# Alighieri1231/WaveformInversionUST

Hardware: NVIDIA B200
Metric: helmholtz_source_solves_per_sec (higher is better)
Workload: dtype c64

## Files before the change

waveforminversionust_b200/csrc/factor.cuh:

```cuda
#pragma once
#include "common.cuh"
#include "gemm_simt.cuh"
#include "gemm_tc2.cuh"
#include "gemm_tc2h.cuh"

namespace ust {

template <typename R>
struct FactorArgs {
    Geom g;
    int phase, step, nbatch;
    const cx<R>* planes;
    cx<R>* T;
    cx<R>* scratch;
    cx<R>* pbuf;
    int* status;
    uint16_t* Rp;
    uint16_t* Xp;
    uint16_t* Cp;
    uint16_t* Pp;
    uint16_t* Tp;
    size_t rp_stride;
    size_t rp2_stride;
    int kb;
// ... 628 lines not shown
    C* Pg = a.pbuf + (size_t)(a.zb0 + z) * GJ_NB * GJ_NB;
    for (int e = tid; e < GJ_NB * GJ_NB; e += 256) Pg[e] = A[(e & 63) * PV_LD + (e >> 6)];
}

template <typename R>
__global__ void __launch_bounds__(256, 1) gj_pivot_kernel(FactorArgs<R> a, int k, int form = 0) {
    extern __shared__ __align__(16) unsigned char smem_raw[];
    pdl_trigger();
    pdl_wait();
    if constexpr (sizeof(R) == 4) {
        if (a.Pp) { gj_pivot_blocked_global(a, k, blockIdx.z, smem_raw, threadIdx.x); return; }
        gj_pivot_body<R>(a, k, blockIdx.z, smem_raw, nullptr);
    } else {
        gj_pivot_blocked_f64(a, k, blockIdx.z, smem_raw, threadIdx.x, form);
    }
}

template <typename R>
constexpr size_t gj_rowpanel_smem() {
    return sizeof(R) == 8 ? 4 * sizeof(double) * GJ_NB * (GJ_NB + 8) : 2 * sizeof(cx<R>) * GJ_NB * GJ_NB;
}
template <typename R>
__global__ void __launch_bounds__(256) gj_rowpanel_kernel(FactorArgs<R> a, int k) {
    extern __shared__ __align__(16) unsigned char smem_raw[];
    const int z = blockIdx.z;
    const int row = chain_row(a.g, a.phase, z, a.step);
    if (row < 0) return;
    const int freq = (a.f0 + chain_freq(a.phase, z));
    const int nP = a.g.nP;
    const cx<R>* __restrict__ Xc = gj_buffer(a, z, freq, row, k);
    cx<R>* __restrict__ Xn = gj_buffer(a, z, freq, row, k + 1);
    const cx<R>* __restrict__ Pg = a.pbuf + (size_t)(a.zb0 + z) * GJ_NB * GJ_NB;
    const int k0 = k * GJ_NB, j0 = blockIdx.x * GJ_NB;
    const int tid = threadIdx.x;
    if constexpr (sizeof(R) == 8) {
        constexpr int LD = GJ_NB + 8;
        double(*Gr)[LD] = reinterpret_cast<double(*)[LD]>(smem_raw);
        double(*Gi)[LD] = Gr + GJ_NB;
        double(*Tr)[LD] = Gi + GJ_NB;
        double(*Ti)[LD] = Tr + GJ_NB;
        for (int e = tid; e < GJ_NB * GJ_NB; e += 256) {
            const int r = e / GJ_NB, c = e % GJ_NB;
            const cx<R> g = Pg[e];
            Gr[r][c] = g.re; Gi[r][c] = g.im;
            cx<R> tv;
            if (j0 == k0) tv = (r == c) ? cxone<R>() : cxzero<R>();
            else tv = Xc[(size_t)(k0 + r) * nP + j0 + c];
            Tr[r][c] = tv.re; Ti[r][c] = tv.im;
        }
        __syncthreads();
        const int lane = tid & 31, warp = tid >> 5;
        const int wm = (warp & 1) * 32, wn = (warp >> 1) * 16, fr = lane >> 2, fk = lane & 3;
        double cr[4][2][2], ci[4][2][2];
#pragma unroll
        for (int i = 0; i < 4; ++i)
#pragma unroll
            for (int j = 0; j < 2; ++j) { cr[i][j][0] = cr[i][j][1] = 0.0; ci[i][j][0] = ci[i][j][1] = 0.0; }
#pragma unroll 4
        for (int k4 = 0; k4 < GJ_NB; k4 += 4) {
            double ar[4], ai[4], br[2], bi[2], nbi[2];
#pragma unroll
            for (int i = 0; i < 4; ++i) { ar[i] = Gr[k4 + fk][wm + 8 * i + fr]; ai[i] = Gi[k4 + fk][wm + 8 * i + fr]; }
#pragma unroll
            for (int j = 0; j < 2; ++j) { br[j] = Tr[k4 + fk][wn + 8 * j + fr]; bi[j] = Ti[k4 + fk][wn + 8 * j + fr]; nbi[j] = -bi[j]; }
#pragma unroll
            for (int i = 0; i < 4; ++i)
#pragma unroll
                for (int j = 0; j < 2; ++j) {
                    dmma884(cr[i][j][0], cr[i][j][1], ar[i], br[j]);
                    dmma884(cr[i][j][0], cr[i][j][1], ai[i], nbi[j]);
                    dmma884(ci[i][j][0], ci[i][j][1], ar[i], bi[j]);
                    dmma884(ci[i][j][0], ci[i][j][1], ai[i], br[j]);
                }
        }
#pragma unroll
        for (int i = 0; i < 4; ++i)
#pragma unroll
            for (int j = 0; j < 2; ++j)
#pragma unroll
                for (int q = 0; q < 2; ++q)
                    Xn[(size_t)(k0 + wm + 8 * i + fr) * nP + j0 + wn + 8 * j + 2 * fk + q] = cx<R>(cr[i][j][q], ci[i][j][q]);
        return;
    } else {
    cx<R>(*G)[GJ_NB] = reinterpret_cast<cx<R>(*)[GJ_NB]>(smem_raw);
    cx<R>(*Tl)[GJ_NB] = reinterpret_cast<cx<R>(*)[GJ_NB]>(smem_raw + sizeof(cx<R>) * GJ_NB * GJ_NB);
    for (int e = tid; e < GJ_NB * GJ_NB; e += 256) {
        int r = e / GJ_NB, c = e % GJ_NB;
        G[r][c] = Pg[e];
        cx<R> tv;
        if (j0 == k0) tv = (r == c) ? cxone<R>() : cxzero<R>();
        else tv = Xc[(size_t)(k0 + r) * nP + j0 + c];
        Tl[r][c] = tv;
    }
    __syncthreads();
    const int tx = tid & 15, ty = tid >> 4;
    cx<R> acc[4][4];
#pragma unroll
    for (int i = 0; i < 4; ++i)
#pragma unroll
        for (int jj = 0; jj < 4; ++jj) acc[i][jj] = cxzero<R>();
#pragma unroll 8
    for (int kk = 0; kk < GJ_NB; ++kk) {
        cx<R> av[4], bv[4];
#pragma unroll
        for (int c = 0; c < 2; ++c) {
            av[2 * c] = G[kk][c * 32 + ty * 2];
            av[2 * c + 1] = G[kk][c * 32 + ty * 2 + 1];
            bv[2 * c] = Tl[kk][c * 32 + tx * 2];
            bv[2 * c + 1] = Tl[kk][c * 32 + tx * 2 + 1];
        }
#pragma unroll
        for (int i = 0; i < 4; ++i)
#pragma unroll
            for (int jj = 0; jj < 4; ++jj) cmac(acc[i][jj], av[i], bv[jj]);
    }
#pragma unroll
    for (int i = 0; i < 4; ++i) {
        int r = (i >> 1) * 32 + ty * 2 + (i & 1);
#pragma unroll
        for (int jj = 0; jj < 4; ++jj) {
            int c = (jj >> 1) * 32 + tx * 2 + (jj & 1);
            Xn[(size_t)(k0 + r) * nP + j0 + c] = acc[i][jj];
        }
    }
    }
}

template <typename R>
__global__ void __launch_bounds__(256) gj_update_kernel(FactorArgs<R> a, int k) {
    __shared__ GemmSmem<R, GJ_NB, GJ_NB> sm;
    const int z = blockIdx.z;
    const int row = chain_row(a.g, a.phase, z, a.step);
    if (row < 0) return;
    const int freq = (a.f0 + chain_freq(a.phase, z));
    const int nP = a.g.nP;
    const cx<R>* Xc = gj_buffer(a, z, freq, row, k);
    cx<R>* Xn = gj_buffer(a, z, freq, row, k + 1);
    const int ib = blockIdx.y + (blockIdx.y >= k ? 1 : 0);
    GemmTile<R> t;
    t.A = Xc + k * GJ_NB; t.lda = nP;
    t.B = Xn + (size_t)k * GJ_NB * nP; t.ldb = nP;
    t.Cin = Xc; t.ldcin = nP;
    t.Cout = Xn; t.ldc = nP;
    t.M = nP; t.N = nP; t.K = GJ_NB; t.Mstore = nP;
    t.m0 = ib * GJ_NB; t.n0 = blockIdx.x * GJ_NB;
    t.mask_lo = k * GJ_NB; t.mask_hi = (k + 1) * GJ_NB;
    t.sgn = R(-1);
    cgemm_tile<R, GJ_NB, GJ_NB, false>(t, sm);
}

__device__ __forceinline__ void gj_colsplit_body(const FactorArgs<float>& a, int k, int z, int bx, int tid) {
    const int row = chain_row(a.g, a.phase, z, a.step);
    if (row < 0) return;
    const int freq = (a.f0 + chain_freq(a.phase, z));
    const int nP = a.g.nP;
    const cx<float>* __restrict__ Xc = gj_buffer(a, z, freq, row, k);
    const int I = bx * 4 + (tid >> 6), J = (tid >> 3) & 7, r = tid & 7;
    const int rr = I * 8 + r;
    if (rr >= nP) return;
    const cx<float>* src = Xc + (size_t)rr * nP + k * GJ_NB + J * 8;
    float re[8], im[8];
#pragma unroll
    for (int c = 0; c < 8; ++c) { cx<float> v = src[c]; re[c] = v.re; im[c] = v.im; }
    uint32_t wr[3][4], wi[3][4];
#pragma unroll
    for (int qd = 0; qd < 4; ++qd) {
        tc::Split3 sr = tc::split2(re[2 * qd], re[2 * qd + 1]);
        tc::Split3 si = tc::split2(im[2 * qd], im[2 * qd + 1]);
#pragma unroll
        for (int sp = 0; sp < 3; ++sp) { wr[sp][qd] = sr.w[sp]; wi[sp][qd] = si.w[sp]; }
    }
    const size_t plane = (size_t)nP * GJ_NB;
    uint16_t* dst = a.Cp + ((size_t)(k & 1) * a.nbmax + a.zb0 + z) * tc2::NPL_A * plane + ((size_t)I * 8 + J) * 64 + r * 8;
#pragma unroll
    for (int sp = 0; sp < 3; ++sp) {
        *reinterpret_cast<uint4*>(dst + sp * plane) = make_uint4(wr[sp][0], wr[sp][1], wr[sp][2], wr[sp][3]);
        *reinterpret_cast<uint4*>(dst + (3 + sp) * plane) = make_uint4(wi[sp][0], wi[sp][1], wi[sp][2], wi[sp][3]);
    }
}

__device__ __forceinline__ void gj_rowsplit_body(const FactorArgs<float>& a, int k, int z, int tn, int r);
__device__ __forceinline__ void gj_colsplit_body(const FactorArgs<float>& a, int k, int z, int bx, int tid);
__global__ void __launch_bounds__(256) gj_k0_kernel(FactorArgs<float> a, int nrow, int ncol, int snap11) {
    extern __shared__ __align__(16) unsigned char smem_raw[];
    pdl_trigger();
    pdl_wait();
    const int z = blockIdx.z, bx = blockIdx.x;
    if (bx < nrow) {
        if (threadIdx.x < 128) gj_rowsplit_body(a, 0, z, bx, threadIdx.x);
    } else if (bx < nrow + ncol) {
        gj_colsplit_body(a, 0, z, bx - nrow, threadIdx.x);
    } else if (snap11 && bx == nrow + ncol) {
        const int row = chain_row(a.g, a.phase, z, a.step);
        if (row < 0) return;
        const int freq = a.f0 + chain_freq(a.phase, z), nP = a.g.nP;
        const cx<float>* __restrict__ Xc = gj_buffer(a, z, freq, row, 0);
        cx<float>* __restrict__ S = a.snap + ((size_t)a.nbmax + a.zb0 + z) * GJ_NB * GJ_NB;
        constexpr int PER = GJ_NB * GJ_NB / 2 / 256;
        float4 v[PER];
#pragma unroll
        for (int j = 0; j < PER; ++j) {
            const int w = threadIdx.x + 256 * j, r = w >> 5, c2 = w & 31;
            v[j] = *reinterpret_cast<const float4*>(Xc + (size_t)(GJ_NB + r) * nP + GJ_NB + 2 * c2);
        }
#pragma unroll
        for (int j = 0; j < PER; ++j) reinterpret_cast<float4*>(S)[threadIdx.x + 256 * j] = v[j];
    } else {
        gj_pivot_blocked_global(a, 0, z, smem_raw, threadIdx.x);
    }
}

__device__ __forceinline__ void gj_rowsplit_body(const FactorArgs<float>& a, int k, int z, int tn, int r) {
    const int row = chain_row(a.g, a.phase, z, a.step);
    if (row < 0) return;
    const int freq = (a.f0 + chain_freq(a.phase, z));
    const int nP = a.g.nP;
    const cx<float>* __restrict__ Xc = gj_buffer(a, z, freq, row, k);
    const int k0 = k * GJ_NB;
    const int n = tn * tc2::TN + r;
    uint16_t* base = a.Xp + ((size_t)(k & 1) * a.nbmax + a.zb0 + z) * a.rp_stride;
    for (int kg = 0; kg < 8; ++kg) {
        float re[8], im[8];
#pragma unroll
        for (int c = 0; c < 8; ++c) {
            cx<float> v = cxzero<float>();
            if (n < nP) {
                if (n >= k0 && n < k0 + GJ_NB) v = cx<float>((n - k0 == 8 * kg + c) ? 1.f : 0.f, 0.f);
                else v = Xc[(size_t)(k0 + 8 * kg + c) * nP + n];
            }
            re[c] = v.re; im[c] = v.im;
        }
        tc2::store_b8(base + ((size_t)tn * (GJ_NB / tc2::KC) + (kg >> 1)) * (tc2::B_STAGE / 2), r, kg & 1, re, im);
    }
}

__device__ __forceinline__ void gj_emit_a(const FactorArgs<float>& a, tc2::Tc2Tile& t, int z, int freq, int row, int k, int row_off) {
    const int nP = a.g.nP, nblk = nP / GJ_NB;
    t.ea_row_off = row_off;
    if (k + 1 < nblk) {
        const size_t plane = (size_t)nP * GJ_NB;
        t.ea_planes = a.Cp + ((size_t)((k + 1) & 1) * a.nbmax + a.zb0 + z) * tc2::NPL_A * plane;
        t.ea_plane_elems = (unsigned)plane; t.ea_nbc = GJ_NB / 8;
        t.ea_n_lo = (k + 1) * GJ_NB; t.ea_n_hi = (k + 2) * GJ_NB; t.ea_col_off = (k + 1) * GJ_NB;
        t.ea_zero_from = 0x7fffffff;
    } else {
        const size_t mat = (size_t)freq * a.g.M + row;
        t.ea_planes = a.Tp + mat * (size_t)tc2::NPL_A * nP * nP;
        t.ea_plane_elems = (unsigned)(nP * nP); t.ea_nbc = nP / 8;
        t.ea_n_lo = 0; t.ea_n_hi = nP; t.ea_col_off = 0;
        t.ea_zero_from = a.g.nI;
    }
}

__device__ __forceinline__ void gj_rowpanel_tile(const FactorArgs<float>& a, int k, int z, int row, int freq, int ntile, float bias_fix,
                                                 const CUtensorMap* pmap, unsigned char* tc2_smem, unsigned long long* trace = nullptr) {
    const int nP = a.g.nP;
    tc2::Tc2Tile t;
    tc2::tile_no_emit(t);
    t.bplanes = a.Xp + ((size_t)(k & 1) * a.nbmax + a.zb0 + z) * a.rp_stride;
    t.amat = (a.pp ? (k & 1) * a.nbmax : 0) + a.zb0 + z;
    t.Cin = nullptr; t.ldcin = nP;
    t.Cout = gj_buffer(a, z, freq, row, k + 1) + (size_t)k * GJ_NB * nP; t.ldc = nP;
    t.M = GJ_NB; t.N = nP; t.K = GJ_NB; t.Mstore = GJ_NB;
    t.m0 = 0; t.n0 = ntile * tc2::TNH;
    t.mask_lo = 0; t.mask_hi = 0; t.skip_lo = 0; t.skip_hi = 0;
    t.sgn = 1.f;
    t.bias_fix = bias_fix;
    t.drain_every = a.gj_drain;
    t.eb_planes = gj_rp(a, k, z); t.eb_m_lo = 0; t.eb_id_lo = 0; t.eb_id_hi = 0;
    gj_emit_a(a, t, z, freq, row, k, k * GJ_NB);
    t.trace = trace;
    tc2::cgemm_tile_h(t, pmap, tc2_smem);
}

__global__ void __launch_bounds__(tc2::NUM_THREADS_H, 2)
tc2_gj_rowpanel_kernel(FactorArgs<float> a, int k, float bias_fix, const __grid_constant__ CUtensorMap pmap) {
    extern __shared__ __align__(1024) unsigned char tc2_smem[];
    constexpr int TW = tc2::TNH;
    pdl_trigger();
    const int z = blockIdx.z;
    const int row = chain_row(a.g, a.phase, z, a.step);
    if (row < 0) { pdl_wait(); return; }
    const int freq = (a.f0 + chain_freq(a.phase, z));
    const int nP = a.g.nP;
    if (blockIdx.x * TW >= nP) {
        pdl_wait();
        const cx<float>* __restrict__ Xc = gj_buffer(a, z, freq, row, k);
        cx<float>* __restrict__ S = a.snap + (size_t)(a.zb0 + z) * GJ_NB * GJ_NB;
        const int k1 = (k + 1) * GJ_NB;
        constexpr int PER = GJ_NB * GJ_NB / 2 / 256;
        float4 v[PER];
#pragma unroll
        for (int j = 0; j < PER; ++j) {
            const int w = threadIdx.x + 256 * j, r = w >> 5, c2 = w & 31;
            v[j] = *reinterpret_cast<const float4*>(Xc + (size_t)(k1 + r) * nP + k1 + 2 * c2);
        }
#pragma unroll
        for (int j = 0; j < PER; ++j) reinterpret_cast<float4*>(S)[threadIdx.x + 256 * j] = v[j];
        return;
    }
    gj_rowpanel_tile(a, k, z, row, freq, blockIdx.x, bias_fix, &pmap, tc2_smem);
}

__global__ void __launch_bounds__(tc2::NUM_THREADS_H, 2)
tc2_gj_update_kernel(FactorArgs<float> a, int k, float bias_fix, int pivot_next, int rp_next, const __grid_constant__ CUtensorMap cmap,
                     const __grid_constant__ CUtensorMap pmap) {
    extern __shared__ __align__(1024) unsigned char tc2_smem[];
    constexpr int TW = tc2::TNH;
    pdl_trigger();
    int bid = blockIdx.x;
    if (pivot_next) {
        if (bid < a.nbatch) {
            {
                static_assert(tc2::CH_LD == GJ_NB + 1, "pivot body reads the staged tile with row stride GJ_NB + 1");
                const int z = bid, kb = k + 1, nP = a.g.nP;
                const int row = chain_row(a.g, a.phase, z, a.step);
                if (row < 0 || (a.exp & 2)) {
                    if (row >= 0 && rp_next && threadIdx.x == 0) atomicExch(gj_flag(a, 0, kb, z), 1);
                    pdl_wait();
                    return;
                }
                tc2::Tc2Tile t;
                tc2::tile_no_emit(t);
                t.bplanes = gj_rp(a, k, z);
                t.amat = (k & 1) * a.nbmax + a.zb0 + z;
                const cx<float>* S1 = a.snap + ((size_t)(a.pp ? (kb & 1) * a.nbmax : 0) + a.zb0 + z) * GJ_NB * GJ_NB;
                t.Cin = S1 - (size_t)(kb * GJ_NB) * GJ_NB - kb * GJ_NB; t.ldcin = GJ_NB;
                t.Cout = nullptr; t.ldc = nP; t.keep = 1;
                t.M = nP; t.N = nP; t.K = GJ_NB; t.Mstore = nP;
                t.m0 = (kb >> 1) * tc2::TM; t.n0 = kb * GJ_NB;
                t.mask_lo = 0; t.mask_hi = 0;
                t.skip_lo = (kb ^ 1) * GJ_NB; t.skip_hi = t.skip_lo + GJ_NB;
                t.sgn = -1.f; t.bias_fix = bias_fix; t.drain_every = a.gj_drain;
                const bool traced = a.trace && a.step == a.trace_step && k == a.trace_k && z < 24;
                if (traced) {
                    t.trace = a.trace + 16 * (1000 + z);
                    if (threadIdx.x == 0) { unsigned smid; asm volatile("mov.u32 %0, %%smid;" : "=r"(smid)); a.trace[16 * 1024 + 1000 + z] = smid; }
                }
                tc2::cgemm_tile_h(t, &cmap, tc2_smem);
                __syncthreads();
                if (a.exp & 1) {
                    if (rp_next && threadIdx.x == 0) atomicExch(gj_flag(a, 0, kb, z), 1);
                    return;
                }
                unsigned char* smem_al = tc2_smem + ((128u - (tc::smem_u32(tc2_smem) & 127u)) & 127u);
                cx<float>* blk = reinterpret_cast<cx<float>*>(smem_al) + (size_t)(kb & 1) * GJ_NB * tc2::CH_LD;
                cx<float>* scr = reinterpret_cast<cx<float>*>(smem_al) + (size_t)tc2::TM * tc2::CH_LD;
                static_assert((size_t)tc2::TM * tc2::CH_LD * sizeof(cx<float>) + gj_pivot2_scratch_bytes <= (size_t)tc2::STAGES_H * tc2::STAGE_H,
                              "pivot scratch must fit behind the staging tile inside the operand ring");
                FactorArgs<float> a2 = a;
                if (a.pp) a2.Pp = a.Pp + (size_t)(kb & 1) * a.nbmax * tc2::NPL_A * GJ_NB * GJ_NB;
                gj_pivot_blocked(a2, z, blk, scr, threadIdx.x, traced ? a.trace + 18 * 1024 + 16 * z : nullptr);
                if (traced && threadIdx.x == 0) a.trace[17 * 1024 + 1000 + z] = tc2::gtime();
                if (rp_next) {
                    __threadfence();
                    __syncthreads();
                    if (threadIdx.x == 0) atomicExch(gj_flag(a, 0, kb, z), 1);
                }
            }
            return;
        }
        bid -= a.nbatch;
    }
    const int nP = a.g.nP, nblk = nP / GJ_NB;
    const int tiles_m = (nP + tc2::TM - 1) / tc2::TM, tiles = (nP + TW - 1) / TW;
    const int ntile_ctas = a.nbatch * tiles_m * tiles;
    if (bid >= ntile_ctas) {
        const int idx = bid - ntile_ctas, z = idx / tiles, ntile = idx % tiles, kn = k + 1;
        const int row = chain_row(a.g, a.phase, z, a.step);
        if (row < 0) { pdl_wait(); return; }
        const int freq = a.f0 + chain_freq(a.phase, z);
        const bool traced = a.trace && a.step == a.trace_step && k == a.trace_k && idx < 96;
        if (traced && threadIdx.x == 0) {
            unsigned smid; asm volatile("mov.u32 %0, %%smid;" : "=r"(smid));
            a.trace[16 * 1024 + 900 + idx] = smid; a.trace[17 * 1024 + 900 + idx] = tc2::gtime();
        }
        pdl_wait();
        if (threadIdx.x == 0) {
            const int* fp = gj_flag(a, 0, kn, z);
            const int* fc = gj_flag(a, 1, kn, z);
            unsigned spins = 0;
            while (ld_acquire_gpu(fp) == 0 || ld_acquire_gpu(fc) < tiles) {
                __nanosleep(100);
                if (++spins > (1u << 22)) __trap();
            }
        }
        __syncthreads();
        asm volatile("fence.proxy.async;" ::: "memory");
        gj_rowpanel_tile(a, kn, z, row, freq, ntile, bias_fix, &pmap, tc2_smem, traced ? a.trace + 16 * (900 + idx) : nullptr);
        return;
    }
    int z, mt, nt;
    const int first = (k + 1) >> 1;
    if (rp_next) {
        const int mt_local = bid / (a.nbatch * tiles), rem = bid % (a.nbatch * tiles);
        z = rem / tiles; nt = rem % tiles;
        mt = mt_local == 0 ? first : (mt_local <= first ? mt_local - 1 : mt_local);
    } else {
        z = bid / (tiles_m * tiles);
        const int rem = bid % (tiles_m * tiles);
        mt = rem / tiles; nt = rem % tiles;
    }
    const int row = chain_row(a.g, a.phase, z, a.step);
    if (row < 0) { pdl_wait(); return; }
    const int freq = (a.f0 + chain_freq(a.phase, z));
    tc2::Tc2Tile t;
    tc2::tile_no_emit(t);
    t.bplanes = gj_rp(a, k, z);
    t.amat = (k & 1) * a.nbmax + a.zb0 + z;
    t.Cin = gj_buffer(a, z, freq, row, k); t.ldcin = nP;
    t.Cout = gj_buffer(a, z, freq, row, k + 1); t.ldc = nP;
    t.M = nP; t.N = nP; t.K = GJ_NB; t.Mstore = nP;
    t.m0 = mt * tc2::TM; t.n0 = nt * TW;
    t.mask_lo = k * GJ_NB; t.mask_hi = (k + 1) * GJ_NB;
    t.skip_lo = k * GJ_NB; t.skip_hi = (k + 1) * GJ_NB;
    t.sgn = -1.f;
    t.bias_fix = bias_fix;
    t.drain_every = a.gj_drain;
    gj_emit_a(a, t, z, freq, row, k, 0);
    if (k + 1 < nblk) {
        t.eb_planes = a.Xp + ((size_t)((k + 1) & 1) * a.nbmax + a.zb0 + z) * a.rp_stride;
        t.eb_m_lo = (k + 1) * GJ_NB; t.eb_id_lo = (k + 1) * GJ_NB; t.eb_id_hi = (k + 2) * GJ_NB;
    }
    if (a.trace && a.step == a.trace_step && k == a.trace_k && bid < 900) {
        t.trace = a.trace + 16 * bid;
        if (threadIdx.x == 0) { unsigned smid; asm volatile("mov.u32 %0, %%smid;" : "=r"(smid)); a.trace[16 * 1024 + bid] = smid; }
    }
    t.prefetch_cin = a.prefetch_cin;
    const int kk = k + 2;
    const bool snap_next = a.pp && kk < nblk && t.m0 == (kk >> 1) * tc2::TM && t.n0 == kk * GJ_NB;
    if (snap_next) t.keep = 1;
    tc2::cgemm_tile_h(t, &cmap, tc2_smem);
    if (snap_next) {
        __syncthreads();
        unsigned char* smem_al = tc2_smem + ((128u - (tc::smem_u32(tc2_smem) & 127u)) & 127u);
        const cx<float>* blk = reinterpret_cast<const cx<float>*>(smem_al) + (size_t)(kk & 1) * GJ_NB * tc2::CH_LD;
        cx<float>* __restrict__ S = a.snap + ((size_t)(kk & 1) * a.nbmax + a.zb0 + z) * GJ_NB * GJ_NB;
#pragma unroll
        for (int j = 0; j < GJ_NB * GJ_NB / tc2::NUM_THREADS_H; ++j) {
            const int e = threadIdx.x + tc2::NUM_THREADS_H * j;
            S[e] = blk[(e >> 6) * tc2::CH_LD + (e & 63)];
        }
    }
    if (rp_next && mt == first) {
        __threadfence();
        __syncthreads();
        if (threadIdx.x == 0) atomicAdd(gj_flag(a, 1, k + 1, z), 1);
    }
}

__global__ void __launch_bounds__(tc2::NUM_THREADS_H, 2)
tc2_gj_pivot_deep_kernel(FactorArgs<float> a, int j, float bias_fix, const __grid_constant__ CUtensorMap pmap, const __grid_constant__ CUtensorMap cmap) {
    extern __shared__ __align__(1024) unsigned char tc2_smem[];
    static_assert(tc2::CH_LD == GJ_NB + 1, "the pivot inversion reads the staged tile with row stride GJ_NB + 1");
    pdl_trigger();
    const int z = blockIdx.x, k = j - 1, nP = a.g.nP;
    const int row = chain_row(a.g, a.phase, z, a.step);
    if (row < 0) { pdl_wait(); return; }
    uint16_t* Rs = a.Rs + (size_t)(a.zb0 + z) * a.rp_stride;
    {
        tc2::Tc2Tile t;
        tc2::tile_no_emit(t);
        t.bplanes = a.Xp + ((size_t)(k & 1) * a.nbmax + a.zb0 + z) * a.rp_stride;
        t.amat = (k & 1) * a.nbmax + a.zb0 + z;
        t.Cin = nullptr; t.ldcin = nP;
        t.Cout = nullptr; t.ldc = nP;
        t.M = GJ_NB; t.N = nP; t.K = GJ_NB; t.Mstore = GJ_NB;
        t.m0 = 0; t.n0 = j * GJ_NB;
        t.mask_lo = 0; t.mask_hi = 0; t.skip_lo = 0; t.skip_hi = 0;
        t.sgn = 1.f; t.bias_fix = bias_fix; t.drain_every = a.gj_drain;
        t.eb_planes = Rs; t.eb_m_lo = 0; t.eb_id_lo = 0; t.eb_id_hi = 0;
        t.tmem_hold = 2;
        tc2::cgemm_tile_h(t, &pmap, tc2_smem);
    }
    __threadfence();
    asm volatile("fence.proxy.async;" ::: "memory");
    __syncthreads();
    tc2::engine_h_release(tc2_smem);
    {
        tc2::Tc2Tile t;
        tc2::tile_no_emit(t);
        t.bplanes = Rs;
        t.amat = (k & 1) * a.nbmax + a.zb0 + z;
        const cx<float>* S1 = a.snap + ((size_t)(j & 1) * a.nbmax + a.zb0 + z) * GJ_NB * GJ_NB;
        t.Cin = S1 - (size_t)(j * GJ_NB) * GJ_NB - j * GJ_NB; t.ldcin = GJ_NB;
        t.Cout = nullptr; t.ldc = nP; t.keep = 1;
        t.M = nP; t.N = nP; t.K = GJ_NB; t.Mstore = nP;
        t.m0 = (j >> 1) * tc2::TM; t.n0 = j * GJ_NB;
        t.mask_lo = 0; t.mask_hi = 0;
        t.skip_lo = (j ^ 1) * GJ_NB; t.skip_hi = t.skip_lo + GJ_NB;
        t.sgn = -1.f; t.bias_fix = bias_fix; t.drain_every = a.gj_drain;
        t.tmem_hold = 1;
        tc2::cgemm_tile_h(t, &cmap, tc2_smem);
    }
    __syncthreads();
    unsigned char* smem_al = tc2_smem + ((128u - (tc::smem_u32(tc2_smem) & 127u)) & 127u);
    cx<float>* blk = reinterpret_cast<cx<float>*>(smem_al) + (size_t)(j & 1) * GJ_NB * tc2::CH_LD;
    cx<float>* scr = reinterpret_cast<cx<float>*>(smem_al) + (size_t)tc2::TM * tc2::CH_LD;
    FactorArgs<float> a2 = a;
    a2.Pp = a.Pp + (size_t)(j & 1) * a.nbmax * tc2::NPL_A * GJ_NB * GJ_NB;
    gj_pivot_blocked(a2, z, blk, scr, threadIdx.x);
}

constexpr int GJ_KB = 128;
enum Gj2Mode { GJ2_MINI = 0, GJ2_FIXA = 1, GJ2_TRAIL = 2 };

__device__ __forceinline__ uint16_t* gj2_cp(const FactorArgs<float>& a, int K, int z) {
    return a.Cp + ((size_t)(K & 1) * a.nbmax + a.zb0 + z) * tc2::NPL_A * (size_t)a.g.nP * GJ_KB;
}
__device__ __forceinline__ void gj2_emit_next(const FactorArgs<float>& a, tc2::Tc2Tile& t, int z, int freq, int row, int K, int row_off) {
    const int nP = a.g.nP, nouter = nP / GJ_KB;
    t.ea_row_off = row_off;
    if (K + 1 < nouter) {
        t.ea_planes = gj2_cp(a, K + 1, z);
        t.ea_plane_elems = (unsigned)(nP * GJ_KB); t.ea_nbc = GJ_KB / 8;
        t.ea_n_lo = (K + 1) * GJ_KB; t.ea_n_hi = (K + 2) * GJ_KB; t.ea_col_off = (K + 1) * GJ_KB;
        t.ea_zero_from = 0x7fffffff;
    } else {
        const size_t mat = (size_t)freq * a.g.M + row;
        t.ea_planes = a.Tp + mat * (size_t)tc2::NPL_A * nP * nP;
        t.ea_plane_elems = (unsigned)(nP * nP); t.ea_nbc = nP / 8;
        t.ea_n_lo = 0; t.ea_n_hi = nP; t.ea_col_off = 0;
        t.ea_zero_from = a.g.nI;
    }
}

__device__ __forceinline__ void gj2_colsplit_body(const FactorArgs<float>& a, int z, int bx, int tid) {
    const int row = chain_row(a.g, a.phase, z, a.step);
    if (row < 0) return;
    const int freq = a.f0 + chain_freq(a.phase, z);
    const int nP = a.g.nP;
    const cx<float>* __restrict__ Xc = gj_buffer(a, z, freq, row, 0);
    const int I = bx * 2 + (tid >> 7), J = (tid >> 3) & 15, r = tid & 7;
    const int rr = I * 8 + r;
    if (rr >= nP) return;
    const cx<float>* src = Xc + (size_t)rr * nP + J * 8;
    float re[8], im[8];
#pragma unroll
    for (int c = 0; c < 8; ++c) { cx<float> v = src[c]; re[c] = v.re; im[c] = v.im; }
    const size_t plane = (size_t)nP * GJ_KB;
    tc2::store_a8(gj2_cp(a, 0, z) + ((size_t)I * (GJ_KB / 8) + J) * 64 + r * 8, plane, re, im);
}

__global__ void __launch_bounds__(256) gj2_k0_kernel(FactorArgs<float> a, int nrow, int ncol) {
    extern __shared__ __align__(16) unsigned char smem_raw[];
    pdl_trigger();
    pdl_wait();
    const int z = blockIdx.z, bx = blockIdx.x;
    if (bx < nrow) {
        if (threadIdx.x < 128) gj_rowsplit_body(a, 0, z, bx, threadIdx.x);
    } else if (bx < nrow + ncol) {
        gj2_colsplit_body(a, z, bx - nrow, threadIdx.x);
    } else {
        gj_pivot_blocked_global(a, 0, z, smem_raw, threadIdx.x);
    }
}

__global__ void __launch_bounds__(tc2::NUM_THREADS_H, 2)
tc2_gj2_rowpanel_kernel(FactorArgs<float> a, int k, float bias_fix, const __grid_constant__ CUtensorMap pmap) {
    extern __shared__ __align__(1024) unsigned char tc2_smem[];
    constexpr int TW = tc2::TNH;
    pdl_trigger();
    const int z = blockIdx.z;
    const int row = chain_row(a.g, a.phase, z, a.step);
    if (row < 0) { pdl_wait(); return; }
    const int freq = a.f0 + chain_freq(a.phase, z);
    const int nP = a.g.nP, K = k >> 1;
    if (blockIdx.x * TW >= nP) {
        pdl_wait();
        const cx<float>* __restrict__ Xc = gj_buffer(a, z, freq, row, k);
        cx<float>* __restrict__ S = a.snap + (size_t)(a.zb0 + z) * GJ_NB * GJ_NB;
        const int k1 = (k + 1) * GJ_NB;
        constexpr int PER = GJ_NB * GJ_NB / 2 / 256;
        float4 v[PER];
#pragma unroll
        for (int j = 0; j < PER; ++j) {
            const int w = threadIdx.x + 256 * j, r = w >> 5, c2 = w & 31;
            v[j] = *reinterpret_cast<const float4*>(Xc + (size_t)(k1 + r) * nP + k1 + 2 * c2);
        }
#pragma unroll
        for (int j = 0; j < PER; ++j) reinterpret_cast<float4*>(S)[threadIdx.x + 256 * j] = v[j];
        return;
    }
    tc2::Tc2Tile t;
    tc2::tile_no_emit(t);
    t.bplanes = a.Xp + ((size_t)(k & 1) * a.nbmax + a.zb0 + z) * a.rp_stride;
    t.amat = a.zb0 + z;
    t.Cin = nullptr; t.ldcin = nP;
    t.Cout = gj_buffer(a, z, freq, row, k) + (size_t)k * GJ_NB * nP; t.ldc = nP;
    t.M = GJ_NB; t.N = nP; t.K = GJ_NB; t.Mstore = GJ_NB;
    t.m0 = 0; t.n0 = blockIdx.x * TW;
    t.mask_lo = 0; t.mask_hi = 0; t.skip_lo = 0; t.skip_hi = 0;
    t.sgn = 1.f;
    t.bias_fix = bias_fix;
    t.drain_every = a.gj_drain;
    t.eb_planes = a.Rp + (size_t)(a.zb0 + z) * a.rp2_stride; t.eb_m_lo = 0; t.eb_id_lo = 0; t.eb_id_hi = 0;
    t.eb_chunks = GJ_KB / tc2::KC; t.eb_chunk0 = (k & 1) * (GJ_NB / tc2::KC);
    if ((k & 1) == 0) {
        t.ea_row_off = k * GJ_NB;
        t.ea_planes = gj2_cp(a, K, z);
        t.ea_plane_elems = (unsigned)(nP * GJ_KB); t.ea_nbc = GJ_KB / 8;
        t.ea_n_lo = (k + 1) * GJ_NB; t.ea_n_hi = (k + 2) * GJ_NB; t.ea_col_off = k * GJ_NB;
        t.ea_zero_from = 0x7fffffff;
    } else {
        gj2_emit_next(a, t, z, freq, row, K, k * GJ_NB);
    }
    tc2::cgemm_tile_h(t, &pmap, tc2_smem);
}

__global__ void __launch_bounds__(tc2::NUM_THREADS_H, 2)
tc2_gj2_update_kernel(FactorArgs<float> a, int k, int mode, float bias_fix, int pivot_next, const __grid_constant__ CUtensorMap cmap) {
    extern __shared__ __align__(1024) unsigned char tc2_smem[];
    constexpr int TW = tc2::TNH;
    pdl_trigger();
    const int nP = a.g.nP, nblk = nP / GJ_NB, K = k >> 1;
    const int ka = 2 * K, kbk = 2 * K + 1;
    int bid = blockIdx.x;
    if (pivot_next) {
        if (bid < a.nbatch) {
            static_assert(tc2::CH_LD == GJ_NB + 1, "the pivot inversion reads the staged tile with row stride GJ_NB + 1");
            const int z = bid, kn = mode == GJ2_MINI ? k + 1 : ka + 2;
            const int row = chain_row(a.g, a.phase, z, a.step);
            if (row < 0 || (a.exp & 2)) { pdl_wait(); return; }
            tc2::Tc2Tile t;
            tc2::tile_no_emit(t);
            t.bplanes = a.Rp + (size_t)(a.zb0 + z) * a.rp2_stride;
            t.b_chunks = GJ_KB / tc2::KC; t.b_chunk0 = 0;
            t.amat = (K & 1) * a.nbmax + a.zb0 + z; t.a_k0 = 0;
            const cx<float>* S1 = a.snap + (size_t)(a.zb0 + z) * GJ_NB * GJ_NB;
            t.Cin = S1 - (size_t)(kn * GJ_NB) * GJ_NB - kn * GJ_NB; t.ldcin = GJ_NB;
            t.Cout = nullptr; t.ldc = nP; t.keep = 1;
            t.M = nP; t.N = nP; t.K = mode == GJ2_MINI ? GJ_NB : GJ_KB; t.Mstore = nP;
            t.m0 = (kn >> 1) * tc2::TM; t.n0 = kn * GJ_NB;
            t.mask_lo = 0; t.mask_hi = 0;
            t.skip_lo = (kn ^ 1) * GJ_NB; t.skip_hi = t.skip_lo + GJ_NB;
            t.sgn = -1.f; t.bias_fix = bias_fix; t.drain_every = a.gj_drain;
            tc2::cgemm_tile_h(t, &cmap, tc2_smem);
            __syncthreads();
            if (a.exp & 1) return;
            unsigned char* smem_al = tc2_smem + ((128u - (tc::smem_u32(tc2_smem) & 127u)) & 127u);
            cx<float>* blk = reinterpret_cast<cx<float>*>(smem_al) + (size_t)(kn & 1) * GJ_NB * tc2::CH_LD;
            cx<float>* scr = reinterpret_cast<cx<float>*>(smem_al) + (size_t)tc2::TM * tc2::CH_LD;
            gj_pivot_blocked(a, z, blk, scr, threadIdx.x);
            return;
        }
        bid -= a.nbatch;
    }
    const int tiles = nP / TW, tiles_m = nP / tc2::TM;
    const int mt_count = mode == GJ2_TRAIL ? tiles_m - 1 : 1;
    const int z = bid / (mt_count * tiles), rem = bid % (mt_count * tiles);
    const int row = chain_row(a.g, a.phase, z, a.step);
    if (row < 0) { pdl_wait(); return; }
    const int freq = a.f0 + chain_freq(a.phase, z);
    int mt = rem / tiles;
    if (mode == GJ2_TRAIL) mt += (mt >= K) ? 1 : 0;
    else mt = K;
    tc2::Tc2Tile t;
    tc2::tile_no_emit(t);
    t.bplanes = a.Rp + (size_t)(a.zb0 + z) * a.rp2_stride;
    t.b_chunks = GJ_KB / tc2::KC;
    t.amat = (K & 1) * a.nbmax + a.zb0 + z;
    t.Cin = gj_buffer(a, z, freq, row, k); t.ldcin = nP;
    t.Cout = gj_buffer(a, z, freq, row, k + 1); t.ldc = nP;
    t.M = nP; t.N = nP; t.Mstore = nP;
    t.m0 = mt * tc2::TM; t.n0 = (rem % tiles) * TW;
    t.sgn = -1.f;
    t.bias_fix = bias_fix;
    t.drain_every = a.gj_drain;
    t.prefetch_cin = a.prefetch_cin;
    if (mode == GJ2_MINI) {
        t.K = GJ_NB; t.a_k0 = 0; t.b_chunk0 = 0;
        t.mask_lo = ka * GJ_NB; t.mask_hi = (ka + 1) * GJ_NB;
        t.skip_lo = ka * GJ_NB; t.skip_hi = (ka + 1) * GJ_NB;
        t.eb_planes = a.Xp + ((size_t)(kbk & 1) * a.nbmax + a.zb0 + z) * a.rp_stride;
        t.eb_m_lo = kbk * GJ_NB; t.eb_id_lo = kbk * GJ_NB; t.eb_id_hi = (kbk + 1) * GJ_NB;
    } else if (mode == GJ2_FIXA) {
        t.K = GJ_NB; t.a_k0 = GJ_NB; t.b_chunk0 = GJ_NB / tc2::KC;
        t.mask_lo = kbk * GJ_NB; t.mask_hi = (kbk + 1) * GJ_NB;
        t.skip_lo = kbk * GJ_NB; t.skip_hi = (kbk + 1) * GJ_NB;
        t.eb_planes = a.Rp + (size_t)(a.zb0 + z) * a.rp2_stride;
        t.eb_chunks = GJ_KB / tc2::KC; t.eb_chunk0 = 0;
        t.eb_m_lo = ka * GJ_NB; t.eb_id_lo = 0; t.eb_id_hi = 0;
        gj2_emit_next(a, t, z, freq, row, K, 0);
    } else {
        t.K = GJ_KB; t.a_k0 = 0; t.b_chunk0 = 0;
        t.mask_lo = ka * GJ_NB; t.mask_hi = (ka + 2) * GJ_NB;
        t.skip_lo = 0; t.skip_hi = 0;
        if (ka + 2 < nblk) {
            t.eb_planes = a.Xp + ((size_t)((ka + 2) & 1) * a.nbmax + a.zb0 + z) * a.rp_stride;
            t.eb_m_lo = (ka + 2) * GJ_NB; t.eb_id_lo = (ka + 2) * GJ_NB; t.eb_id_hi = (ka + 3) * GJ_NB;
        }
        gj2_emit_next(a, t, z, freq, row, K, 0);
    }
    tc2::cgemm_tile_h(t, &cmap, tc2_smem);
}

}
```

waveforminversionust_b200/csrc/gemm_tc2h.cuh:

```cuda
#pragma once
#include "gemm_tc2.cuh"

namespace ust {
namespace tc2 {

constexpr int TNH = 64;
constexpr int BH_PLANE = 2 * TNH * KC * 2;
constexpr int BH_STAGE = NPL_B * BH_PLANE;
constexpr int STAGE_H = A_STAGE + BH_STAGE;
constexpr int STAGES_H = 3;
constexpr int NUM_THREADS_H = 256;
constexpr int NUM_WARPS_H = 8;
constexpr int CH_LD = TNH + 1;
constexpr int SMEM_BYTES_H = STAGES_H * STAGE_H + 128 + 128 + 384;
static_assert(TM * CH_LD * 8 <= STAGES_H * STAGE_H, "epilogue staging tile must fit in the operand ring");
static_assert(2 * (SMEM_BYTES_H + 1024) <= 227 * 1024, "two CTAs per SM");
constexpr uint32_t TMEM_COLS_H = 256;
constexpr uint32_t IDESC_N64 = IDESC_BASE | ((64u >> 3) << 17);

__device__ __forceinline__ void engine_h_release(unsigned char* smem_raw) {
    __syncthreads();
    if (threadIdx.x == 0) {
        const uint32_t smem_base = (smem_u32(smem_raw) + 127u) & ~127u;
        const uint32_t bar_base = smem_base + STAGES_H * STAGE_H;
        for (int i = 0; i < 2 * STAGES_H + 3; ++i) asm volatile("mbarrier.inval.shared::cta.b64 [%0];" ::"r"(bar_base + 8u * i) : "memory");
    }
    __syncthreads();
}

__device__ __forceinline__ void cgemm_tile_h(const Tc2Tile& t_in, const CUtensorMap* amap, unsigned char* smem_raw) {
    typedef cx<float> C;
    const int tid = threadIdx.x, warp = tid >> 5, lane = tid & 31;
    if (warp == 0) TC2_TRACE(0);
    if (tid == 0) asm volatile("prefetch.tensormap [%0];" ::"l"((uint64_t)amap) : "memory");
    const uint32_t smem_base = (smem_u32(smem_raw) + 127u) & ~127u;
    unsigned char* smem_al = smem_raw + (smem_base - smem_u32(smem_raw));
    const uint32_t bar_base = smem_base + STAGES_H * STAGE_H;
    auto full_bar = [&](int s) { return bar_base + 8u * s; };
    auto empty_bar = [&](int s) { return bar_base + 8u * (STAGES_H + s); };
    const uint32_t d1_full = bar_base + 8u * (2 * STAGES_H);
    const uint32_t d1_empty = bar_base + 8u * (2 * STAGES_H + 1);
    const uint32_t d2_full = bar_base + 8u * (2 * STAGES_H + 2);
    const uint32_t tmem_slot = bar_base + 8u * (2 * STAGES_H + 3);
    volatile uint32_t* tmem_slot_ptr = reinterpret_cast<volatile uint32_t*>(smem_al + (tmem_slot - smem_base));
    Tc2Tile* t_sh = reinterpret_cast<Tc2Tile*>(smem_al + STAGES_H * STAGE_H + 128);
    if (tid == 0) *t_sh = t_in;
    const Tc2Tile& t = *t_sh;

    if (warp == 2) {
        if (lane == 0) {
            for (int s = 0; s < STAGES_H; ++s) { mbar_init(full_bar(s), 1); mbar_init(empty_bar(s), 2); }
            mbar_init(d1_full, 1);
            mbar_init(d1_empty, NUM_WARPS_H);
            mbar_init(d2_full, 1);
            asm volatile("fence.mbarrier_init.release.cluster;" ::: "memory");
        }
        __syncwarp();
        if (!(t_in.tmem_hold & 1)) {
            asm volatile("tcgen05.alloc.cta_group::1.sync.aligned.shared::cta.b32 [%0], %1;" ::"r"(tmem_slot), "r"(TMEM_COLS_H) : "memory");
            asm volatile("tcgen05.relinquish_alloc_permit.cta_group::1.sync.aligned;" ::: "memory");
        }
    }
    asm volatile("tcgen05.fence::before_thread_sync;" ::: "memory");
    __syncthreads();
    asm volatile("tcgen05.fence::after_thread_sync;" ::: "memory");
    const uint32_t tmem_acc = *tmem_slot_ptr;
    pdl_wait();
    if (warp == 0) TC2_TRACE(1);
    const uint32_t D1 = tmem_acc, D2 = tmem_acc + 2 * TNH;
    const int nk = (t.K + KC - 1) / KC;
    const int D = t.drain_every < 1 ? 1 : (t.drain_every > nk ? nk : t.drain_every);

    const int bch = t.b_chunks > 0 ? t.b_chunks : nk;
    const unsigned char* bsrc = reinterpret_cast<const unsigned char*>(t.bplanes) + ((size_t)(t.n0 / TN) * bch + t.b_chunk0) * B_STAGE + ((t.n0 % TN) / TNH) * 2048;
    const int am0 = t.m0, amat = t.amat, ak0 = t.a_k0;
    auto load_chunk = [&](int c) {
        const int s = c % STAGES_H;
        const uint32_t sa = smem_base + s * STAGE_H, sb = sa + A_STAGE;
        mbar_expect_tx_e(full_bar(s), STAGE_H);
        tma_load_5d_e(sa, amap, full_bar(s), 0, (ak0 + c * KC) >> 3, am0 >> 3, 0, amat);
        const unsigned char* bc = bsrc + (size_t)c * B_STAGE;
#pragma unroll
        for (int p = 0; p < NPL_B; ++p) {
            bulk_load_e(sb + p * BH_PLANE, bc + p * B_PLANE, 2048, full_bar(s));
            bulk_load_e(sb + p * BH_PLANE + 2048, bc + p * B_PLANE + 4096, 2048, full_bar(s));
        }
    };
    if (warp == 0) {
        load_chunk(0);
        TC2_TRACE(2);
    } else if (warp == 2) {
        for (int c = 1; c < nk && c < STAGES_H; ++c) load_chunk(c);
    }
    if (t.Cin && tid >= 128 && t.prefetch_cin) {
        const int rr = tid - 128, m = t.m0 + rr;
        const int ncols = t.N - t.n0 < TNH ? t.N - t.n0 : TNH;
        if (m < t.Mstore && !(m >= t.skip_lo && m < t.skip_hi) && ncols > 0 && ((ncols * 8) & 15) == 0 && ((t.ldcin & 1) == 0) && ((t.n0 & 1) == 0))
            asm volatile("cp.async.bulk.prefetch.L2.global [%0], %1;" ::"l"((uint64_t)(t.Cin + (size_t)m * t.ldcin + t.n0)), "r"((uint32_t)(ncols * 8)) : "memory");
    }

    const uint32_t id1 = IDESC_N128, id2 = IDESC_N64 | IDESC_ANEG, id3 = IDESC_N64;
    uint64_t dAr[3], dAi[3], dB[3], dBi[3];
#pragma unroll
    for (int i = 0; i < 3; ++i) {
        dAr[i] = make_desc(smem_base + i * A_PLANE, 128u, 256u);
        dAi[i] = make_desc(smem_base + (3 + i) * A_PLANE, 128u, 256u);
        dB[i] = make_desc(smem_base + A_STAGE + i * BH_PLANE, 128u, 256u);
        dBi[i] = make_desc(smem_base + A_STAGE + i * BH_PLANE + (TNH / 8) * 256, 128u, 256u);
    }
    auto issue = [&](uint32_t d, uint64_t so, int i, int j, uint32_t acc_first) {
        umma_e(d, dAr[i] + so, dB[j] + so, id1, acc_first);
        umma_e(d, dAi[i] + so, dBi[j] + so, id2, 1u);
        umma_e(d + TNH, dAi[i] + so, dB[j] + so, id3, 1u);
    };

    const int q = warp & 3, cg = warp >> 2;
    const uint32_t lane_addr = ((uint32_t)(q * 32)) << 16;
    float acc_re[32], acc_im[32];
#pragma unroll
    for (int j = 0; j < 32; ++j) { acc_re[j] = 0.f; acc_im[j] = 0.f; }

    for (int c = 0; c < nk; ++c) {
        const int s = c % STAGES_H;
        const uint32_t use = (uint32_t)(c / STAGES_H);
        if (warp < 2) {
            const uint64_t so = (uint64_t)((uint32_t)(s * STAGE_H) >> 4);
            mbar_wait(full_bar(s), use & 1u);
            if (warp == 0) {
                if (c == 0) TC2_TRACE(3);
                if (c > 0 && c % D == 0) mbar_wait(d1_empty, (uint32_t)(c / D - 1) & 1u);
                if (c == nk - 1) TC2_TRACE(8);
                asm volatile("tcgen05.fence::after_thread_sync;" ::: "memory");
                issue(D1, so, 0, 0, c % D == 0 ? 0u : 1u);
                if ((c + 1) % D == 0 || c == nk - 1) umma_commit_e(d1_full);
                umma_commit_e(empty_bar(s));
                if (c == 0) TC2_TRACE(4);
            } else {
                asm volatile("tcgen05.fence::after_thread_sync;" ::: "memory");
                issue(D2, so, 0, 1, c > 0 ? 1u : 0u);
                issue(D2, so, 1, 0, 1u);
                issue(D2, so, 0, 2, 1u);
                issue(D2, so, 2, 0, 1u);
                issue(D2, so, 1, 1, 1u);
                umma_commit_e(empty_bar(s));
                if (c == nk - 1) { TC2_TRACE(9); umma_commit_e(d2_full); }
            }
            __syncwarp();
        }
        if ((c + 1) % D == 0 || c == nk - 1) {
        mbar_wait(d1_full, (uint32_t)(c / D) & 1u);
        if (warp == 3 && c == 0) TC2_TRACE(5);
        asm volatile("tcgen05.fence::after_thread_sync;" ::: "memory");
#pragma unroll
        for (int h = 0; h < 4; ++h) {
            uint32_t vr[8], vi[8];
            tmem_ld8(D1 + lane_addr + (uint32_t)(32 * cg + 8 * h), vr);
            tmem_ld8(D1 + lane_addr + (uint32_t)(TNH + 32 * cg + 8 * h), vi);
            asm volatile("tcgen05.wait::ld.sync.aligned;" ::: "memory");
            if (h == 3) {
                asm volatile("tcgen05.fence::before_thread_sync;" ::: "memory");
                __syncwarp();
                if (lane == 0) mbar_arrive(d1_empty);
                if (warp == 3 && c == 0) TC2_TRACE(6);
            }
#pragma unroll
            for (int j = 0; j < 8; ++j) {
                acc_re[8 * h + j] += __uint_as_float(vr[j]);
                acc_im[8 * h + j] += __uint_as_float(vi[j]);
            }
        }
        }
        if (warp == 0 && c + STAGES_H < nk) {
            mbar_wait(empty_bar(s), use & 1u);
            load_chunk(c + STAGES_H);
        }
    }
    mbar_wait(d2_full, 0);
    if (warp == 3) TC2_TRACE(10);
    asm volatile("tcgen05.fence::after_thread_sync;" ::: "memory");
    C* stage = reinterpret_cast<C*>(smem_al);
    {
        const int r = q * 32 + lane;
        const float bias = t.bias_fix * (float)D;
#pragma unroll
        for (int h = 0; h < 4; ++h) {
            uint32_t vr[8], vi[8];
            tmem_ld8(D2 + lane_addr + (uint32_t)(32 * cg + 8 * h), vr);
            tmem_ld8(D2 + lane_addr + (uint32_t)(TNH + 32 * cg + 8 * h), vi);
            asm volatile("tcgen05.wait::ld.sync.aligned;" ::: "memory");
#pragma unroll
            for (int j = 0; j < 8; ++j) {
                const float ar = acc_re[8 * h + j], ai = acc_im[8 * h + j];
                const float cr = fmaf(ar, bias, __uint_as_float(vr[j]));
                const float ci = fmaf(ai, bias, __uint_as_float(vi[j]));
                stage[(size_t)r * CH_LD + 32 * cg + 8 * h + j] = C(ar + cr, ai + ci);
            }
        }
    }
    if (warp == 3) TC2_TRACE(11);
    asm volatile("tcgen05.fence::before_thread_sync;" ::: "memory");
    __syncthreads();
    if (warp == 2 && !(t_in.tmem_hold & 2)) {
        asm volatile("tcgen05.fence::after_thread_sync;" ::: "memory");
        asm volatile("tcgen05.dealloc.cta_group::1.sync.aligned.b32 %0, %1;" ::"r"(tmem_acc), "r"(TMEM_COLS_H) : "memory");
    }
    if (warp == 3) TC2_TRACE(15);
    const Tc2Tile tl = *t_sh;
    const bool emit = tl.ea_planes != nullptr || tl.eb_planes != nullptr || tl.keep;
    const bool vec_ok = ((tl.ldc & 1) == 0) && ((((uintptr_t)tl.Cout) & 15) == 0) && (tl.n0 % 2 == 0) &&
                        (!tl.Cin || (((tl.ldcin & 1) == 0) && ((((uintptr_t)tl.Cin) & 15) == 0)));
    if (vec_ok && tl.n0 + TNH <= tl.N) {
        constexpr int RPW = TM / NUM_WARPS_H;
        float4 cin[RPW];
        unsigned live = 0;
        const int nloc = lane * 2, n = tl.n0 + nloc;
#pragma unroll
        for (int j = 0; j < RPW; ++j) {
            const int m = tl.m0 + warp + NUM_WARPS_H * j;
            const bool lv = m < tl.Mstore && !(m >= tl.skip_lo && m < tl.skip_hi);
            live |= (lv ? 1u : 0u) << j;
            cin[j] = make_float4(0.f, 0.f, 0.f, 0.f);
            if (lv && tl.Cin) cin[j] = *reinterpret_cast<const float4*>(tl.Cin + (size_t)m * tl.ldcin + n);
        }
        const bool z0 = n >= tl.mask_lo && n < tl.mask_hi, z1 = n + 1 >= tl.mask_lo && n + 1 < tl.mask_hi;
#pragma unroll
        for (int j = 0; j < RPW; ++j) {
            const int rr = warp + NUM_WARPS_H * j;
            const int m = tl.m0 + rr;
            if (!((live >> j) & 1u)) continue;
            const C a0 = stage[(size_t)rr * CH_LD + nloc], a1 = stage[(size_t)rr * CH_LD + nloc + 1];
            float4 c = cin[j];
            if (z0) { c.x = 0.f; c.y = 0.f; }
            if (z1) { c.z = 0.f; c.w = 0.f; }
            c.x += tl.sgn * a0.re; c.y += tl.sgn * a0.im; c.z += tl.sgn * a1.re; c.w += tl.sgn * a1.im;
            if (tl.Cout) *reinterpret_cast<float4*>(tl.Cout + (size_t)m * tl.ldc + n) = c;
            if (emit) { stage[(size_t)rr * CH_LD + nloc] = C(c.x, c.y); stage[(size_t)rr * CH_LD + nloc + 1] = C(c.z, c.w); }
        }
    } else {
        for (int rr = warp; rr < TM; rr += NUM_WARPS_H) {
            const int m = tl.m0 + rr;
            if (m >= tl.Mstore || (m >= tl.skip_lo && m < tl.skip_hi)) continue;
            const int nloc = lane * 2, n = tl.n0 + nloc;
            if (n >= tl.N) continue;
            const C a0 = stage[(size_t)rr * CH_LD + nloc], a1 = stage[(size_t)rr * CH_LD + nloc + 1];
            C c0 = cxzero<float>(), c1 = cxzero<float>();
            if (tl.Cin) {
                const C* ci = tl.Cin + (size_t)m * tl.ldcin + n;
                c0 = ci[0];
                if (n + 1 < tl.N) c1 = ci[1];
                if (n >= tl.mask_lo && n < tl.mask_hi) c0 = cxzero<float>();
                if (n + 1 >= tl.mask_lo && n + 1 < tl.mask_hi) c1 = cxzero<float>();
            }
            c0.re += tl.sgn * a0.re; c0.im += tl.sgn * a0.im;
            c1.re += tl.sgn * a1.re; c1.im += tl.sgn * a1.im;
            if (tl.Cout) {
                C* co = tl.Cout + (size_t)m * tl.ldc + n;
                co[0] = c0;
                if (n + 1 < tl.N) co[1] = c1;
            }
            if (emit) { stage[(size_t)rr * CH_LD + nloc] = c0; stage[(size_t)rr * CH_LD + nloc + 1] = c1; }
        }
    }
    if (warp == 3) TC2_TRACE(12);
    if (emit) {
        __syncthreads();
        if (tl.eb_planes && tl.eb_m_lo >= tl.m0 && tl.eb_m_lo < tl.m0 + TM) {
            const int r0 = tl.eb_m_lo - tl.m0;
#pragma unroll
            for (int h = 0; h < 2; ++h) {
                const int e = tid + NUM_THREADS_H * h;
                const int nloc = e & (TNH - 1), kg = e >> 6;
                const int n = tl.n0 + nloc;
                float re[8], im[8];
#pragma unroll
                for (int c = 0; c < 8; ++c) {
                    C v = stage[(size_t)(r0 + 8 * kg + c) * CH_LD + nloc];
                    if (n >= tl.eb_id_lo && n < tl.eb_id_hi) v = C((n - tl.eb_id_lo == 8 * kg + c) ? 1.f : 0.f, 0.f);
                    if (n >= tl.N) v = cxzero<float>();
                    re[c] = v.re; im[c] = v.im;
                }
                const int ech = tl.eb_chunks > 0 ? tl.eb_chunks : 64 / KC;
                uint16_t* chunk = tl.eb_planes + ((size_t)(n / TN) * ech + tl.eb_chunk0 + (kg >> 1)) * (B_STAGE / 2);
                store_b8(chunk, n % TN, kg & 1, re, im);
            }
        }
        if (tl.ea_planes) {
            const int lo = tl.ea_n_lo > tl.n0 ? tl.ea_n_lo : tl.n0;
            const int hi = tl.ea_n_hi < tl.n0 + TNH ? tl.ea_n_hi : tl.n0 + TNH;
            const int nJ = hi > lo ? (hi - lo) >> 3 : 0;
            for (int e = tid; e < nJ * TM; e += NUM_THREADS_H) {
                const int rr = e & (TM - 1), jj = e >> 7;
                const int m = tl.m0 + rr;
                if (m >= tl.Mstore || (m >= tl.skip_lo && m < tl.skip_hi)) continue;
                const int n8 = lo + 8 * jj;
                const int tr = m + tl.ea_row_off, tcol = n8 - tl.ea_col_off;
                float re[8], im[8];
#pragma unroll
                for (int c = 0; c < 8; ++c) {
                    C v = stage[(size_t)rr * CH_LD + (n8 - tl.n0) + c];
                    if (tr >= tl.ea_zero_from || tcol + c >= tl.ea_zero_from || n8 + c >= tl.N) v = cxzero<float>();
                    re[c] = v.re; im[c] = v.im;
                }
                uint16_t* dst = tl.ea_planes + ((size_t)(tr >> 3) * tl.ea_nbc + (tcol >> 3)) * 64 + (tr & 7) * 8;
                store_a8(dst, tl.ea_plane_elems, re, im);
            }
        }
    }
    if (warp == 3) TC2_TRACE(13);
    if (warp == 2) TC2_TRACE(14);
}

}
}
```

waveforminversionust_b200/csrc/ustfwi.cu:

```cuda
#include "../../include/ustfwi.h"

#include <math.h>
#include <stdlib.h>
#include <string.h>

#include <algorithm>
#include <map>
#include <mutex>
#include <vector>

#include "assemble.cuh"
#include "common.cuh"
#include "factor.cuh"
#include "fwi.cuh"
#include "sweep.cuh"

namespace ust {
static thread_local std::string g_err;
thread_local long long g_launches = 0;
bool g_use_pdl = true;
thread_local bool g_pdl_batch_ok = true;
void set_error(const std::string& s) { g_err = s; }
}

using namespace ust;

struct ust_plan {
    ust_plan_desc d;
    Geom g;
    size_t rsz, csz;
    double h = 0, gr = 1, a0 = 0, Lpml = 0;
    bool grid_set = false, acq_set = false, factored = false;
    bool use_tc2 = false;
    bool t_ring = false;
    int prefetch_cin = 1;
    static constexpr int MAX_GROUPS = 8;
    int ngroups = 2;
    cudaStream_t side[MAX_GROUPS] = {};
    cudaEvent_t ev_fork = nullptr, ev_join[MAX_GROUPS] = {};
    bool deep = false;
    cudaStream_t pivst[MAX_GROUPS] = {};
    cudaEvent_t ev_upd[MAX_GROUPS] = {}, ev_piv[MAX_GROUPS][2] = {};
    uint16_t* Rs = nullptr;
    bool fuse = false;
    int* gj_flags = nullptr;
    uint16_t *Tp = nullptr, *Wp = nullptr;
    void* snap = nullptr;
    uint16_t *Rp = nullptr, *Cp = nullptr, *Xp = nullptr, *Pp = nullptr;
    size_t rp_stride = 0, rp2_stride = 0;
    bool gj2 = false;
    CUtensorMap cmaps[2], cmaps2[2], pmaps[2];
    size_t wp_stride = 0;
    int kpad = 0;
    int gj_drain = 1, sweep_drain = 1;
    float bias_fix = 2.5e-8f;
    CUtensorMap amaps[2];
    int nfreq_cur = 0;
    std::vector<double> freqs_cur;
    size_t bytes = 0;
    int num_sms = 148;
    void *exn = nullptr, *rexh = nullptr, *eyn = nullptr, *reyh = nullptr;
    double *d_vminmax = nullptr, *d_freqs = nullptr, *d_bde = nullptr, *d_scal = nullptr, *d_invv2 = nullptr;
    double* d_sig2 = nullptr;
    int* d_status = nullptr;
    void *planes = nullptr, *T = nullptr, *scratch = nullptr, *W = nullptr, *pbuf = nullptr;
    void *vel = nullptr, *U = nullptr, *Lam = nullptr, *src_est = nullptr, *Xh = nullptr;
    void *slow_h2d = nullptr, *rec_h2d = nullptr, *grad_d2h = nullptr;
    int *src_lin = nullptr, *rx_lin = nullptr, *mask = nullptr;
    int nt = 0, nelem = 0, nm = 0;
    bool onehot_ok = false;
    short first_row[8], last_row[8];
    void *slow_in = nullptr, *rec_in = nullptr, *grad_out = nullptr, *sd_in = nullptr;
    void *v_in = nullptr, *hv_out = nullptr, *drec = nullptr;
    void *kappa_in = nullptr, *grad_kappa_out = nullptr;
    void *kappa_h2d = nullptr, *grad_kappa_d2h = nullptr;
    bool fwi_done = false;
    bool lossy = false;
    bool gn_ok = false;
    bool use_graphs = true;
    struct GraphEntry { cudaGraphExec_t exec = nullptr; long long launches = 0; };
    std::map<long long, GraphEntry> graphs;
    cudaEvent_t ev_in = nullptr, ev_out = nullptr;
    double* h_stage = nullptr;
    cudaStream_t own_stream = nullptr;
    unsigned long long* trace = nullptr;
    int trace_step = -1, trace_k = -1;
    bool schur_pivot0 = true;
    int pdl_min_batch = 8;
    int active_groups = 1;
    int eval_nfreq = 1;
    int ksplit_ok = 2;
    int exp = 0;
    bool lookahead = true;
    bool prof = false;
    std::vector<cudaEvent_t> ev;
    std::vector<int> ev_cls;
    size_t ev_used = 0;
};

struct ProfScope {
    ust_plan* p; long idx; cudaStream_t st;
    ProfScope(ust_plan* p_, int cls, cudaStream_t st_) : p(p_), idx(-1), st(st_) {
        if (p->prof && p->ev_used + 2 <= p->ev.size()) {
            idx = (long)p->ev_used; p->ev_used += 2; p->ev_cls[idx / 2] = cls;
            cudaEventRecord(p->ev[idx], st);
        }
    }
    ~ProfScope() { if (idx >= 0) cudaEventRecord(p->ev[idx + 1], st); }
};
enum ProfClass { PC_ASSEMBLE = 0, PC_SCHUR, PC_GJ_PANEL, PC_GJ_UPDATE, PC_TRI_APPLY, PC_SWEEP_GEMM, PC_RECEIVER, PC_GRADIENT, PC_T_SPLIT, PC_GJ_PIVOT, PC_GJ_ROWPANEL, PC_GJ_K0, PC_COUNT };

static int dev_alloc(ust_plan* p, void** ptr, size_t bytes) {
    UST_CUDA(cudaMalloc(ptr, bytes));
    p->bytes += bytes;
    return 0;
}

static int check_plan(const ust_plan* p) {
    if (!p) { set_error("null plan"); return 1; }
    return 0;
}

static int dump_update_trace(ust_plan* p, cudaStream_t st) {
    std::vector<unsigned long long> h(19 * 1024);
    UST_CUDA(cudaStreamSynchronize(st));
    UST_CUDA(cudaMemcpy(h.data(), p->trace, h.size() * sizeof(unsigned long long), cudaMemcpyDeviceToHost));
    unsigned long long t0 = ~0ull;
    for (int b = 0; b < 1024; ++b) if (h[16 * b] && h[16 * b] < t0) t0 = h[16 * b];
    for (int b = 0; b < 1024; ++b) {
        if (!h[16 * b]) continue;
        fprintf(stderr, "upd cta %4d sm %3d:", b, (int)h[16 * 1024 + b]);
        for (int i = 0; i < 16; ++i) fprintf(stderr, " %lld", h[16 * b + i] ? (long long)(h[16 * b + i] - t0) : -1LL);
        fprintf(stderr, " %lld", h[17 * 1024 + b] ? (long long)(h[17 * 1024 + b] - t0) : -1LL);
        if (b >= 1000 && b < 1024)
            for (int i = 0; i < 13; ++i) fprintf(stderr, " %lld", h[18 * 1024 + 16 * (b - 1000) + i] ? (long long)(h[18 * 1024 + 16 * (b - 1000) + i] - t0) : -1LL);
        fprintf(stderr, "\n");
    }
    UST_CUDA(cudaMemset(p->trace, 0, h.size() * sizeof(unsigned long long)));
    return 0;
}

static void drop_graphs(ust_plan* p) {
    for (auto& kv : p->graphs)
        if (kv.second.exec) cudaGraphExecDestroy(kv.second.exec);
    p->graphs.clear();
}

template <typename R>
static int set_grid_impl(ust_plan* p, const double* x, const double* y, double a0, double L) {
    const int Nx = p->g.Nx, Ny = p->g.Ny;
    double h = (x[Nx - 1] - x[0]) / (Nx - 1), gh = (y[Ny - 1] - y[0]) / (Ny - 1);
    p->h = h; p->gr = gh / h; p->a0 = a0; p->Lpml = L;
    auto prof = [&](const double* c, int n, std::vector<cx<R>>& node, std::vector<cx<R>>& rhalf) {
        double cmin = c[0], cmax = c[n - 1];
        double ctr = 0.5 * (cmin + cmax), span = 0.5 * (cmax - cmin);
        node.resize(n); rhalf.resize(n);
        for (int i = 0; i < 2 * n - 1; ++i) {
            double xe = cmin + (cmax - cmin) * (double)i / (double)(2 * (n - 1));
            double s = fmax(fabs(xe - ctr) - span + L, 0.0) / L;
            double im = -a0 * s * s;
            if ((i & 1) == 0) node[i / 2] = cx<R>((R)1.0, (R)im);
            else {
                double d = 1.0 + im * im;
                rhalf[i / 2] = cx<R>((R)(1.0 / d), (R)(-im / d));
            }
        }
        rhalf[n - 1] = cx<R>((R)0, (R)0);
    };
    std::vector<cx<R>> exn, rexh, eyn, reyh;
    prof(x, Nx, exn, rexh);
    prof(y, Ny, eyn, reyh);
    UST_CUDA(cudaMemcpy(p->exn, exn.data(), Nx * sizeof(cx<R>), cudaMemcpyHostToDevice));
    UST_CUDA(cudaMemcpy(p->rexh, rexh.data(), Nx * sizeof(cx<R>), cudaMemcpyHostToDevice));
    UST_CUDA(cudaMemcpy(p->eyn, eyn.data(), Ny * sizeof(cx<R>), cudaMemcpyHostToDevice));
    UST_CUDA(cudaMemcpy(p->reyh, reyh.data(), Ny * sizeof(cx<R>), cudaMemcpyHostToDevice));
    p->grid_set = true;
    p->factored = false;
    return 0;
}

template <typename R>
static int gj_invert_batch(ust_plan* p, int phase, int step, int f0, int nf, cudaStream_t st, int gidx) {
    const Geom& g = p->g;
    const int nbatch = phase == PH_CHAIN ? 2 * nf : nf;
    FactorArgs<R> a;
    a.g = g; a.phase = phase; a.step = step; a.nbatch = nbatch;
    a.f0 = f0; a.zb0 = 2 * f0; a.t_ring = p->t_ring ? 1 : 0;
    ust::g_pdl_batch_ok = nbatch * p->active_groups > p->pdl_min_batch ||
                          (long long)nbatch * p->active_groups * cdiv_i(g.nP, tc2::TM) * (g.nP / tc2::TNH) > 2LL * p->num_sms;
    a.planes = (const cx<R>*)p->planes; a.T = (cx<R>*)p->T; a.scratch = (cx<R>*)p->scratch; a.pbuf = (cx<R>*)p->pbuf; a.status = p->d_status;
    a.Rp = p->Rp; a.Cp = p->Cp; a.Xp = p->Xp; a.Pp = p->Pp; a.Tp = p->Tp; a.rp_stride = p->rp_stride; a.nbmax = 2 * p->d.max_freq;
    a.rp2_stride = p->rp2_stride; a.kb = p->gj2 ? GJ_KB : GJ_NB;
    a.inplace = p->use_tc2 ? 1 : 0; a.gj_drain = p->gj_drain; a.snap = (cx<R>*)p->snap;
    a.trace = p->trace; a.trace_step = p->trace_step; a.trace_k = p->trace_k;
    a.prefetch_cin = p->prefetch_cin; a.exp = p->exp;
    a.deep = (p->deep && g.nP / GJ_NB > 1) ? 1 : 0; a.Rs = p->Rs;
    a.fuse = (p->fuse && !p->deep && p->lookahead && g.nP / GJ_NB > 1 && g.nP / GJ_NB <= GJ_MAXBLK) ? 1 : 0;
    a.pp = (a.deep || a.fuse) ? 1 : 0; a.flags = p->gj_flags;
    const int nblk = g.nP / GJ_NB;
    {
        dim3 grid(cdiv_i(g.nP, SchurTile<R>::TS), cdiv_i(g.nP, SchurTile<R>::TS), nbatch), block(16, 16);
        const int pivot0 = (sizeof(R) == 4 && p->use_tc2 && p->schur_pivot0) ? 1 : 0;
        ProfScope ps(p, PC_SCHUR, st);
        UST_CUDA(launch_pdl(schur_kernel<R>, grid, block, pivot0 ? gj_pivot2_scratch_bytes : 0, st, a, pivot0));
        UST_LAUNCH_CHECK();
    }
    const size_t smem = gj_rowpanel_smem<R>();
    if constexpr (sizeof(R) == 4) {
        if (p->use_tc2 && p->gj2) {
            {
                ProfScope ps(p, PC_GJ_K0, st);
                const int nrow = cdiv_i(g.nP, tc2::TN), ncol = g.nP / 16;
                UST_CUDA(launch_pdl(gj2_k0_kernel, dim3(nrow + ncol + (p->schur_pivot0 ? 0 : 1), 1, nbatch), dim3(256), gj_pivot2_smem_bytes, st, a, nrow, ncol));
            }
            UST_LAUNCH_CHECK();
            const int tiles_h = g.nP / tc2::TNH, tiles_m = g.nP / tc2::TM;
            auto rowpanel = [&](int k) -> int {
                if (p->exp & 4) return 0;
                ProfScope ps(p, PC_GJ_ROWPANEL, st);
                const int snap_cta = (k + 1 < nblk) ? 1 : 0;
                UST_CUDA(launch_pdl(tc2_gj2_rowpanel_kernel, dim3(tiles_h + snap_cta, 1, nbatch), dim3(tc2::NUM_THREADS_H), tc2::SMEM_BYTES_H, st, a, k, p->bias_fix, p->pmaps[0]));
                UST_LAUNCH_CHECK();
                return 0;
            };
            auto update = [&](int k, int mode, int mt_count, int pivot_next) -> int {
                ProfScope ps(p, mode == GJ2_TRAIL ? PC_GJ_UPDATE : (mode == GJ2_MINI ? PC_GJ_PANEL : PC_GJ_PIVOT), st);
                UST_CUDA(launch_pdl(tc2_gj2_update_kernel, dim3(nbatch * mt_count * tiles_h + (pivot_next ? nbatch : 0)), dim3(tc2::NUM_THREADS_H),
                                    tc2::SMEM_BYTES_H, st, a, k, mode, p->bias_fix, pivot_next, p->cmaps2[0]));
                UST_LAUNCH_CHECK();
                return 0;
            };
            for (int K = 0; K < nblk / 2; ++K) {
                const int ka = 2 * K, kbk = ka + 1;
                UST_TRY(rowpanel(ka));
                UST_TRY(update(ka, GJ2_MINI, 1, 1));
                UST_TRY(rowpanel(kbk));
                UST_TRY(update(kbk, GJ2_FIXA, 1, 0));
                if (tiles_m > 1) UST_TRY(update(ka, GJ2_TRAIL, tiles_m - 1, ka + 2 < nblk ? 1 : 0));
            }
            return 0;
        }
        if (p->use_tc2) {
            const bool deep = a.deep != 0;
            {
                ProfScope ps(p, PC_GJ_K0, st);
                const int nrow = cdiv_i(g.nP, tc2::TN), ncol = nblk > 1 ? cdiv_i(g.nP, 32) : 0;
                UST_CUDA(launch_pdl(gj_k0_kernel, dim3(nrow + ncol + (a.pp ? 1 : 0) + (p->schur_pivot0 ? 0 : 1), 1, nbatch), dim3(256), gj_pivot2_smem_bytes, st, a, nrow, ncol, a.pp));
            }
            UST_LAUNCH_CHECK();
            const bool la = p->lookahead && nblk > 1 && !deep;
            const int tiles = cdiv_i(g.nP, tc2::TN), tiles_h = cdiv_i(g.nP, tc2::TNH);
            cudaStream_t ps_st = p->pivst[gidx];
            auto pivot_deep = [&](int j) -> int {
                UST_CUDA(cudaEventRecord(p->ev_upd[gidx], st));
                UST_CUDA(cudaStreamWaitEvent(ps_st, p->ev_upd[gidx], 0));
                {
                    ProfScope p1(p, PC_GJ_PIVOT, ps_st);
                    UST_CUDA(launch_pdl(tc2_gj_pivot_deep_kernel, dim3(nbatch), dim3(tc2::NUM_THREADS_H), tc2::SMEM_BYTES_H, ps_st, a, j, p->bias_fix, p->pmaps[0], p->cmaps[0]));
                }
                UST_LAUNCH_CHECK();
                UST_CUDA(cudaEventRecord(p->ev_piv[gidx][j & 1], ps_st));
                return 0;
            };
            if (deep) UST_TRY(pivot_deep(1));
            for (int k = 0; k < nblk; ++k) {
                {
                    ProfScope ps(p, PC_GJ_PANEL, st);
                    if (k > 0 && !la && !deep) {
                        ProfScope p1(p, PC_GJ_PIVOT, st);
                        UST_CUDA(launch_pdl(gj_pivot_kernel<R>, dim3(1, 1, nbatch), dim3(256), gj_pivot2_smem_bytes, st, a, k, 0));
                        UST_LAUNCH_CHECK();
                    }
                    if (k > 0 && deep) UST_CUDA(cudaStreamWaitEvent(st, p->ev_piv[gidx][k & 1], 0));
                    if (!(p->exp & 4) && (!a.fuse || k == 0)) {
                        ProfScope p2(p, PC_GJ_ROWPANEL, st);
                        const int snap_cta = (la && !a.pp && k + 1 < nblk) ? 1 : 0;
                        UST_CUDA(launch_pdl(tc2_gj_rowpanel_kernel, dim3(tiles_h + snap_cta, 1, nbatch), dim3(tc2::NUM_THREADS_H), tc2::SMEM_BYTES_H, st, a, k, p->bias_fix, p->pmaps[0]));
                    }
                    UST_LAUNCH_CHECK();
                }
                if (nblk > 1) {
                    const int pivot_next = (la && k + 1 < nblk) ? 1 : 0;
                    const int rp_next = (a.fuse && k + 1 < nblk && !(p->exp & 4)) ? 1 : 0;
                    ProfScope ps(p, PC_GJ_UPDATE, st);
                    UST_CUDA(launch_pdl(tc2_gj_update_kernel, dim3(nbatch * tiles * tiles_h + (pivot_next ? nbatch : 0) + (rp_next ? nbatch * tiles_h : 0)), dim3(tc2::NUM_THREADS_H),
                                        tc2::SMEM_BYTES_H, st, a, k, p->bias_fix, pivot_next, rp_next, p->cmaps[0], p->pmaps[0]));
                    UST_LAUNCH_CHECK();
                }
                if (deep && k + 2 < nblk) UST_TRY(pivot_deep(k + 2));
            }
            return 0;
        }
    }
    const bool la64 = sizeof(R) == 8 && p->lookahead && nblk > 1 && p->pivst[gidx] != nullptr;
    const size_t piv_smem = sizeof(R) == 8 ? gj_pivot_f64_smem_bytes : gj_pivot_smem<R>();
    for (int k = 0; k < nblk; ++k) {
        {
            ProfScope ps(p, PC_GJ_PANEL, st);
            if (k == 0 || !la64) {
                ProfScope p1(p, PC_GJ_PIVOT, st);
                gj_pivot_kernel<R><<<dim3(1, 1, nbatch), 256, piv_smem, st>>>(a, k, 0);
            } else {
                UST_CUDA(cudaStreamWaitEvent(st, p->ev_piv[gidx][k & 1], 0));
            }
            UST_LAUNCH_CHECK();
            {
                ProfScope p2(p, PC_GJ_ROWPANEL, st);
                gj_rowpanel_kernel<R><<<dim3(nblk, 1, nbatch), 256, smem, st>>>(a, k);
            }
            UST_LAUNCH_CHECK();
        }
        if (la64 && k + 1 < nblk) {
            cudaStream_t ps_st = p->pivst[gidx];
            UST_CUDA(cudaEventRecord(p->ev_upd[gidx], st));
            UST_CUDA(cudaStreamWaitEvent(ps_st, p->ev_upd[gidx], 0));
            {
                ProfScope p1(p, PC_GJ_PIVOT, ps_st);
                gj_pivot_kernel<R><<<dim3(1, 1, nbatch), 256, piv_smem, ps_st>>>(a, k + 1, 1);
            }
            UST_LAUNCH_CHECK();
            UST_CUDA(cudaEventRecord(p->ev_piv[gidx][(k + 1) & 1], ps_st));
        }
        if (nblk > 1) {
            {
                ProfScope ps(p, PC_GJ_UPDATE, st);
                gj_update_kernel<R><<<dim3(nblk, nblk - 1, nbatch), 256, 0, st>>>(a, k);
            }
            UST_LAUNCH_CHECK();
        }
    }
    return 0;
}

static int upload_params(ust_plan* p, int nfreq, const double* freqs, const double* bde, cudaStream_t st) {
    if (!p->grid_set) { set_error("ust_factor: ust_plan_set_grid has not been called"); return 1; }
    if (nfreq < 1 || nfreq > p->d.max_freq) { set_error("ust_factor: nfreq out of range"); return 1; }
    UST_CUDA(cudaMemcpyAsync(p->d_freqs, freqs, nfreq * sizeof(double), cudaMemcpyHostToDevice, st));
    if (bde) UST_CUDA(cudaMemcpyAsync(p->d_bde, bde, 3 * nfreq * sizeof(double), cudaMemcpyHostToDevice, st));
    p->freqs_cur.assign(freqs, freqs + nfreq);
    return 0;
}

struct Group { int f0, nf; cudaStream_t st; int idx; };

static std::vector<Group> make_groups(ust_plan* p, int f_begin, int nfreq, cudaStream_t main_st, bool allow_split = true) {
    int G = std::min(std::min(p->ngroups, nfreq / 4), (int)ust_plan::MAX_GROUPS);
    if (p->prof || !allow_split || G < 1) G = 1;
    p->active_groups = G;
    p->eval_nfreq = nfreq;
    std::vector<Group> gs;
    for (int i = 0; i < G; ++i) {
        const int lo = (int)((long long)nfreq * i / G), hi = (int)((long long)nfreq * (i + 1) / G);
        gs.push_back({f_begin + lo, hi - lo, i == 0 ? main_st : p->side[i], i});
    }
    return gs;
}
static int fork_groups(ust_plan* p, const std::vector<Group>& gs) {
    if (gs.size() < 2) return 0;
    UST_CUDA(cudaEventRecord(p->ev_fork, gs[0].st));
    for (size_t i = 1; i < gs.size(); ++i) UST_CUDA(cudaStreamWaitEvent(gs[i].st, p->ev_fork, 0));
    return 0;
}
static int join_groups(ust_plan* p, const std::vector<Group>& gs) {
    for (size_t i = 1; i < gs.size(); ++i) {
        UST_CUDA(cudaEventRecord(p->ev_join[i], gs[i].st));
        UST_CUDA(cudaStreamWaitEvent(gs[0].st, p->ev_join[i], 0));
    }
    return 0;
}

template <typename R>
static int factor_prologue(ust_plan* p, const void* vel_dev, int nfreq, bool has_bde, cudaStream_t st, const void* kappa_dev = nullptr) {
    const Geom& g = p->g;
    if (!has_bde) {
        minmax_kernel<R><<<1, 1024, 0, st>>>((const R*)vel_dev, g.N, p->d_vminmax);
        UST_LAUNCH_CHECK();
        stencil_params_kernel<<<nfreq, 1024, 0, st>>>(p->d_vminmax, p->d_freqs, p->h, p->gr, p->d_bde);
        UST_LAUNCH_CHECK();
    }
    UST_CUDA(cudaMemsetAsync(p->d_status, 0, sizeof(int), st));
    if (kappa_dev) sig2_kernel<R><<<(unsigned)((g.N + 255) / 256), 256, 0, st>>>((const R*)vel_dev, (const R*)kappa_dev, (double2*)p->d_sig2, g.N);
    else inv_v2_kernel<R><<<(unsigned)((g.N + 255) / 256), 256, 0, st>>>((const R*)vel_dev, p->d_invv2, g.N);
    UST_LAUNCH_CHECK();
    return 0;
}

template <typename R>
static int factor_groups(ust_plan* p, const void* vel_dev, const std::vector<Group>& gs, bool lossy = false) {
    const Geom& g = p->g;
    AsmArgs aa;
    aa.g = g; aa.h = p->h; aa.gr = p->gr; aa.stencil = p->d.stencil; aa.exp = (p->exp & 8) ? 1 : 0;
    for (const Group& q : gs)
        for (int c0 = 0; c0 < q.nf; c0 += ASM_MAXF) {
            const int f0 = q.f0 + c0;
            aa.nfreq = std::min(q.nf - c0, (int)ASM_MAXF);
            ProfScope ps(p, PC_ASSEMBLE, q.st);
            const dim3 grid(cdiv_i(g.Nx, 256), g.Ny);
            if (lossy)
                assemble_kernel<R, true><<<grid, 256, 0, q.st>>>(
                    aa, p->d_sig2, (const cx<R>*)p->exn, (const cx<R>*)p->rexh, (const cx<R>*)p->eyn, (const cx<R>*)p->reyh,
                    p->d_freqs + f0, p->d_bde + 3 * f0, (cx<R>*)p->planes + (size_t)f0 * 9 * g.N);
            else
                assemble_kernel<R, false><<<grid, 256, 0, q.st>>>(
                    aa, p->d_invv2, (const cx<R>*)p->exn, (const cx<R>*)p->rexh, (const cx<R>*)p->eyn, (const cx<R>*)p->reyh,
                    p->d_freqs + f0, p->d_bde + 3 * f0, (cx<R>*)p->planes + (size_t)f0 * 9 * g.N);
            UST_LAUNCH_CHECK();
        }
    const int len = std::max(g.mid, g.M - 1 - g.mid);
    for (int s = 0; s < len; ++s)
        for (const Group& q : gs) UST_TRY(gj_invert_batch<R>(p, PH_CHAIN, s, q.f0, q.nf, q.st, q.idx));
    for (const Group& q : gs) UST_TRY(gj_invert_batch<R>(p, PH_MID, 0, q.f0, q.nf, q.st, q.idx));
    return 0;
}

template <typename R>
static int factor_enqueue(ust_plan* p, const void* vel_dev, int nfreq, bool has_bde, cudaStream_t st, const void* kappa_dev) {
    UST_TRY(factor_prologue<R>(p, vel_dev, nfreq, has_bde, st, kappa_dev));
    const std::vector<Group> gs = make_groups(p, 0, nfreq, st);
    UST_TRY(fork_groups(p, gs));
    UST_TRY(factor_groups<R>(p, vel_dev, gs, kappa_dev != nullptr));
    UST_TRY(join_groups(p, gs));
    p->nfreq_cur = nfreq;
    p->factored = true;
    return 0;
}

template <typename R>
static int factor_impl(ust_plan* p, const void* vel_dev, int nfreq, const double* freqs, const double* bde, cudaStream_t st,
                       const void* kappa_dev = nullptr) {
    p->gn_ok = false;
    UST_TRY(upload_params(p, nfreq, freqs, bde, st));
    if (kappa_dev) p->lossy = true;
    return factor_enqueue<R>(p, vel_dev, nfreq, bde != nullptr, st, kappa_dev);
}

template <typename R, int BM, int BN>
static int launch_sweep_gemm(ust_plan* p, const SweepArgs<R>& s, dim3 grid, cudaStream_t st) {
    {
        ProfScope ps(p, PC_SWEEP_GEMM, st);
        if (s.adjoint) sweep_gemm_kernel<R, BM, BN, true><<<grid, 256, 0, st>>>(s);
        else sweep_gemm_kernel<R, BM, BN, false><<<grid, 256, 0, st>>>(s);
    }
    UST_LAUNCH_CHECK();
    return 0;
}

template <typename R>
static int sweep_step(ust_plan* p, SweepArgs<R>& s, cudaStream_t st) {
    const Geom& g = p->g;
    const long long elems = (long long)g.nI * s.nrhs;
    ust::g_pdl_batch_ok = s.nbatch * p->active_groups > p->pdl_min_batch;
    if constexpr (sizeof(R) == 4) {
        if (p->use_tc2) {
            Tc2SweepExtra x;
            x.Wp = p->Wp + (size_t)2 * s.f0 * p->wp_stride;
            x.wp_stride = p->wp_stride; x.kpad = p->kpad; x.bias_fix = p->bias_fix; x.drain_every = p->sweep_drain;
            x.prefetch_cin = p->prefetch_cin; x.ksplit = 1;
            {
                ProfScope ps(p, PC_TRI_APPLY, st);
                UST_CUDA(launch_pdl(tri_apply2_kernel, dim3(p->kpad / 8, cdiv_i(s.nrhs, tc2::TN), s.nbatch), dim3(128), 0, st, s, x));
            }
            UST_LAUNCH_CHECK();
            dim3 grid(cdiv_i(s.nrhs, tc2::TN), cdiv_i(g.nI, tc2::TM), s.nbatch);
            const long long all_tiles = 2LL * p->eval_nfreq * grid.x * grid.y;
            const int nchunks = p->kpad / tc2::KC;
            x.ksplit = 1;
            if (p->ksplit_ok >= 2 && 2 * all_tiles <= p->num_sms && nchunks >= 8) x.ksplit = 2;
            if (p->ksplit_ok >= 4 && 4 * all_tiles <= p->num_sms && nchunks >= 16) x.ksplit = 4;
            {
                ProfScope ps(p, PC_SWEEP_GEMM, st);
                if (x.ksplit > 1) {
                    grid.x *= x.ksplit;
                    if (s.adjoint) UST_CUDA(launch_pdl_cluster(tc2_sweep_gemm_kernel<true>, grid, dim3(tc2::NUM_THREADS), tc2::SMEM_BYTES, st, (unsigned)x.ksplit, s, x, p->amaps[1]));
                    else UST_CUDA(launch_pdl_cluster(tc2_sweep_gemm_kernel<false>, grid, dim3(tc2::NUM_THREADS), tc2::SMEM_BYTES, st, (unsigned)x.ksplit, s, x, p->amaps[0]));
                } else if (s.adjoint) UST_CUDA(launch_pdl(tc2_sweep_gemm_kernel<true>, grid, dim3(tc2::NUM_THREADS), tc2::SMEM_BYTES, st, s, x, p->amaps[1]));
                else UST_CUDA(launch_pdl(tc2_sweep_gemm_kernel<false>, grid, dim3(tc2::NUM_THREADS), tc2::SMEM_BYTES, st, s, x, p->amaps[0]));
            }
            UST_LAUNCH_CHECK();
            return 0;
        }
    }
    {
        ProfScope ps(p, PC_TRI_APPLY, st);
        tri_apply_kernel<R><<<dim3((unsigned)((elems + 255) / 256), 1, s.nbatch), 256, 0, st>>>(s);
    }
    UST_LAUNCH_CHECK();
    const int bn = s.nrhs > 32 ? 64 : 32;
    int bm = 64;
    if ((long long)cdiv_i(g.nI, 64) * cdiv_i(s.nrhs, bn) * s.nbatch < p->num_sms) bm = 32;
    dim3 grid(cdiv_i(s.nrhs, bn), cdiv_i(g.nI, bm), s.nbatch);
    if (bm == 64 && bn == 64) return launch_sweep_gemm<R, 64, 64>(p, s, grid, st);
    if (bm == 32 && bn == 64) return launch_sweep_gemm<R, 32, 64>(p, s, grid, st);
    if (bm == 64 && bn == 32) return launch_sweep_gemm<R, 64, 32>(p, s, grid, st);
    return launch_sweep_gemm<R, 32, 32>(p, s, grid, st);
}

template <typename R>
static int sweeps_groups(ust_plan* p, const std::vector<Group>& gs, cx<R>* X, size_t x_stride, int nrhs, int adjoint, bool onehot = false) {
    const Geom& g = p->g;
    std::vector<SweepArgs<R>> sv(gs.size());
    for (size_t i = 0; i < gs.size(); ++i) {
        SweepArgs<R>& s = sv[i];
        const int f0 = gs[i].f0;
        s.g = g; s.adjoint = adjoint; s.nrhs = nrhs;
        s.onehot = (onehot && p->onehot_ok) ? 1 : 0;
        for (int j = 0; j < 8; ++j) { s.first_row[j] = p->first_row[j]; s.last_row[j] = p->last_row[j]; }
        s.planes = (const cx<R>*)p->planes + (size_t)f0 * 9 * g.N;
        s.T = (const cx<R>*)p->T + (size_t)f0 * g.M * (size_t)g.nP * g.nP;
        s.W = (cx<R>*)p->W + (size_t)2 * f0 * g.nP * p->d.max_nrhs;
        s.X = X + (size_t)f0 * x_stride; s.x_stride = x_stride; s.f0 = f0;
    }
    const int len = std::max(g.mid, g.M - 1 - g.mid);
    for (int step = 0; step < len; ++step)
        for (size_t i = 0; i < gs.size(); ++i) {
            SweepArgs<R>& s = sv[i];
            s.mode = SW_ELIM; s.phase = PH_CHAIN; s.nbatch = 2 * gs[i].nf; s.step = step;
            UST_TRY(sweep_step<R>(p, s, gs[i].st));
        }
    for (size_t i = 0; i < gs.size(); ++i) {
        SweepArgs<R>& s = sv[i];
        s.mode = SW_ELIM; s.phase = PH_MID; s.nbatch = gs[i].nf; s.step = 0;
        UST_TRY(sweep_step<R>(p, s, gs[i].st));
    }
    for (int step = len - 1; step >= 0; --step)
        for (size_t i = 0; i < gs.size(); ++i) {
            SweepArgs<R>& s = sv[i];
            s.mode = SW_BACK; s.phase = PH_CHAIN; s.nbatch = 2 * gs[i].nf; s.step = step;
            UST_TRY(sweep_step<R>(p, s, gs[i].st));
        }
    return 0;
}

template <typename R>
static int ring_fix(ust_plan* p, int ifreq, cx<R>* X, int nrhs, int adjoint, bool before, cudaStream_t st) {
    const Geom& g = p->g;
    const cx<R>* planes_f = (const cx<R>*)p->planes + (size_t)ifreq * 9 * g.N;
    if (!adjoint && before) {
        int count = 2 * g.nI + 2 * std::max(g.M - 2, 0);
        long long th = (long long)count * nrhs;
        ring_pre_kernel<R><<<(unsigned)((th + 255) / 256), 256, 0, st>>>(g, planes_f, X, nrhs, count);
        UST_LAUNCH_CHECK();
    } else if (adjoint && !before) {
        int count = 2 * g.Nx + 2 * (g.Ny - 2);
        long long th = (long long)count * nrhs;
        ring_post_adj_kernel<R><<<(unsigned)((th + 255) / 256), 256, 0, st>>>(g, planes_f, X, nrhs, count);
        UST_LAUNCH_CHECK();
    }
    return 0;
}

template <typename R>
static int solve_impl(ust_plan* p, int ifreq, void* X, int nrhs, int adjoint, cudaStream_t st) {
    if (!p->factored) { set_error("ust_solve: no factorisation (call ust_factor first)"); return 1; }
    if (ifreq < 0 || ifreq >= p->nfreq_cur) { set_error("ust_solve: ifreq out of range"); return 1; }
    if (nrhs < 1 || nrhs > p->d.max_nrhs) { set_error("ust_solve: nrhs exceeds plan max_nrhs"); return 1; }
    UST_TRY(ring_fix<R>(p, ifreq, (cx<R>*)X, nrhs, adjoint, true, st));
    const std::vector<Group> one = {{ifreq, 1, st}};
    UST_TRY(sweeps_groups<R>(p, one, (cx<R>*)X, 0, nrhs, adjoint));
    UST_TRY(ring_fix<R>(p, ifreq, (cx<R>*)X, nrhs, adjoint, false, st));
    return 0;
}

template <bool TA>
__global__ void __launch_bounds__(tc2::NUM_THREADS, 1) tc2_test_gemm_kernel(tc2::Tc2Tile t, const __grid_constant__ CUtensorMap amap) {
    extern __shared__ __align__(1024) unsigned char tc2_smem[];
    t.m0 = blockIdx.y * tc2::TM; t.n0 = blockIdx.x * tc2::TN;
    if (blockIdx.x | blockIdx.y | blockIdx.z) t.trace = nullptr;
    tc2::cgemm_tile<TA>(t, &amap, tc2_smem);
}
__global__ void __launch_bounds__(tc2::NUM_THREADS_H, 2) tc2h_test_gemm_kernel(tc2::Tc2Tile t, const __grid_constant__ CUtensorMap amap) {
    extern __shared__ __align__(1024) unsigned char tc2_smem[];
    t.m0 = blockIdx.y * tc2::TM; t.n0 = blockIdx.x * tc2::TNH;
    if (blockIdx.x | blockIdx.y | blockIdx.z) t.trace = nullptr;
    tc2::cgemm_tile_h(t, &amap, tc2_smem);
}
template <bool TA>
__global__ void __launch_bounds__(256) simt_test_gemm_kernel(GemmTile<float> t) {
    __shared__ GemmSmem<float, 64, 64> sm;
    t.m0 = blockIdx.y * 64; t.n0 = blockIdx.x * 64;
    cgemm_tile<float, 64, 64, TA>(t, sm);
}

__global__ void pack_f32x2_kernel(const double* __restrict__ in, float* __restrict__ out, int n) {
    const int i = blockIdx.x * blockDim.x + threadIdx.x;
    if (i >= n) return;
    const double v = in[i];
    const float hi = (float)v;
    out[2 * i] = hi;
    out[2 * i + 1] = (float)(v - (double)hi);
}

template <typename R>
__global__ void recip_kernel(const R* __restrict__ in, R* __restrict__ out, long long n) {
    long long i = (long long)blockIdx.x * blockDim.x + threadIdx.x;
    if (i < n) out[i] = R(1) / in[i];
}

template <typename R>
static int fwi_enqueue(ust_plan* p, int nfreq, bool has_bde, cudaStream_t st, bool lossy = false) {
    const Geom& g = p->g;
    const int nt = p->nt;
    const size_t stride = (size_t)g.N * nt;
    const void* slow = p->slow_in;
    double* loss_dev = p->d_scal;
    recip_kernel<R><<<(unsigned)((g.N + 255) / 256), 256, 0, st>>>((const R*)slow, (R*)p->vel, g.N);
    UST_LAUNCH_CHECK();
    UST_TRY(factor_prologue<R>(p, p->vel, nfreq, has_bde, st, lossy ? p->kappa_in : nullptr));
    UST_CUDA(cudaMemsetAsync(loss_dev, 0, sizeof(double), st));
    const std::vector<Group> gs = make_groups(p, 0, nfreq, st);
    UST_TRY(fork_groups(p, gs));
    UST_TRY(factor_groups<R>(p, p->vel, gs, lossy));
    for (const Group& q : gs) {
        cx<R>* Uq = (cx<R>*)p->U + (size_t)q.f0 * stride;
        UST_CUDA(cudaMemsetAsync(Uq, 0, stride * q.nf * sizeof(cx<R>), q.st));
        onehot_scatter_kernel<R><<<cdiv_i(nt * q.nf, 256), 256, 0, q.st>>>(Uq, stride, p->src_lin, nt, q.nf);
        UST_LAUNCH_CHECK();
    }
    UST_TRY(sweeps_groups<R>(p, gs, (cx<R>*)p->U, stride, nt, 0, true));
    for (const Group& q : gs) {
        UST_CUDA(cudaMemsetAsync((cx<R>*)p->Lam + (size_t)q.f0 * stride, 0, stride * q.nf * sizeof(cx<R>), q.st));
        RecvArgs<R> ra;
        ra.U = (const cx<R>*)p->U + (size_t)q.f0 * stride; ra.Lam = (cx<R>*)p->Lam + (size_t)q.f0 * stride; ra.stride_f = stride;
        ra.rec = (const cx<R>*)p->rec_in + (size_t)q.f0 * nt * p->nelem;
        ra.rx_lin = p->rx_lin; ra.mask = p->mask; ra.src_est = (cx<R>*)p->src_est + (size_t)q.f0 * nt; ra.loss = loss_dev;
        ra.nt = nt; ra.nm = p->nm; ra.nelem = p->nelem;
        ProfScope ps(p, PC_RECEIVER, q.st);
        receiver_kernel<R><<<dim3(nt, q.nf), 256, 0, q.st>>>(ra);
        UST_LAUNCH_CHECK();
    }
    UST_TRY(sweeps_groups<R>(p, gs, (cx<R>*)p->Lam, stride, nt, 1));
    for (const Group& q : gs)
        for (int f = q.f0; f < q.f0 + q.nf; ++f) UST_TRY(ring_fix<R>(p, f, (cx<R>*)p->Lam + (size_t)f * stride, nt, 1, false, q.st));
    UST_TRY(join_groups(p, gs));
    GradArgs<R> ga;
    ga.U = (const cx<R>*)p->U; ga.Lam = (const cx<R>*)p->Lam; ga.stride_f = stride; ga.src_est = (const cx<R>*)p->src_est;
    ga.freqs = p->d_freqs; ga.slow = (const R*)slow; ga.grad = (R*)p->grad_out; ga.N = g.N; ga.nt = nt; ga.nfreq = nfreq;
    ga.kappa = (const R*)p->kappa_in; ga.grad_kappa = (R*)p->grad_kappa_out;
    const int blocks = (int)std::min<long long>((g.N + 7) / 8, (long long)p->num_sms * 8);
    {
        ProfScope ps(p, PC_GRADIENT, st);
        if (lossy) gradient_kernel<R, true><<<blocks, 256, 0, st>>>(ga);
        else gradient_kernel<R, false><<<blocks, 256, 0, st>>>(ga);
    }
    UST_LAUNCH_CHECK();
    return 0;
}

template <typename R>
static int linesearch_enqueue(ust_plan* p, cudaStream_t st) {
    const Geom& g = p->g;
    const int nt = p->nt, nfreq = p->nfreq_cur;
    const size_t stride = (size_t)g.N * nt;
    double* out2 = p->d_scal + 2;
    UST_CUDA(cudaMemsetAsync(out2, 0, 2 * sizeof(double), st));
    const std::vector<Group> gs = make_groups(p, 0, nfreq, st);
    UST_TRY(fork_groups(p, gs));
    for (const Group& q : gs) {
        PertArgs<R> pa;
        pa.U = (const cx<R>*)p->U + (size_t)q.f0 * stride; pa.Out = (cx<R>*)p->Lam + (size_t)q.f0 * stride; pa.stride_f = stride;
        pa.src_est = (const cx<R>*)p->src_est + (size_t)q.f0 * nt;
        pa.freqs = p->d_freqs + q.f0; pa.slow = (const R*)p->slow_in; pa.sd = (const R*)p->sd_in; pa.N = g.N; pa.nt = nt; pa.nfreq = q.nf;
        pert_rhs_kernel<R><<<dim3(p->num_sms * 4, q.nf), 256, 0, q.st>>>(pa);
        UST_LAUNCH_CHECK();
    }
    UST_TRY(sweeps_groups<R>(p, gs, (cx<R>*)p->Lam, stride, nt, 0));
    for (const Group& q : gs) {
        LineArgs<R> la;
        la.U = (const cx<R>*)p->U + (size_t)q.f0 * stride; la.Pert = (const cx<R>*)p->Lam + (size_t)q.f0 * stride; la.stride_f = stride;
        la.rec = (const cx<R>*)p->rec_in + (size_t)q.f0 * nt * p->nelem;
        la.rx_lin = p->rx_lin; la.mask = p->mask; la.src_est = (const cx<R>*)p->src_est + (size_t)q.f0 * nt; la.out2 = out2;
        la.nt = nt; la.nm = p->nm; la.nelem = p->nelem;
        linesearch_kernel<R><<<dim3(nt, q.nf), 256, 0, q.st>>>(la);
        UST_LAUNCH_CHECK();
    }
    UST_TRY(join_groups(p, gs));
    return 0;
}

template <typename R>
static int gn_hvp_enqueue(ust_plan* p, cudaStream_t st) {
    const Geom& g = p->g;
    const int nt = p->nt, nfreq = p->nfreq_cur;
    const size_t stride = (size_t)g.N * nt;
    double* jv2 = p->d_scal + 6;
    UST_CUDA(cudaMemsetAsync(jv2, 0, sizeof(double), st));
    const std::vector<Group> gs = make_groups(p, 0, nfreq, st);
    UST_TRY(fork_groups(p, gs));
    for (const Group& q : gs) {
        PertArgs<R> pa;
        pa.U = (const cx<R>*)p->U + (size_t)q.f0 * stride; pa.Out = (cx<R>*)p->Lam + (size_t)q.f0 * stride; pa.stride_f = stride;
        pa.src_est = (const cx<R>*)p->src_est + (size_t)q.f0 * nt;
        pa.freqs = p->d_freqs + q.f0; pa.slow = (const R*)p->slow_in; pa.sd = (const R*)p->v_in; pa.N = g.N; pa.nt = nt; pa.nfreq = q.nf;
        pert_rhs_kernel<R><<<dim3(p->num_sms * 4, q.nf), 256, 0, q.st>>>(pa);
        UST_LAUNCH_CHECK();
    }
    UST_TRY(sweeps_groups<R>(p, gs, (cx<R>*)p->Lam, stride, nt, 0));
    for (const Group& q : gs) {
        GnRecvArgs<R> ra;
        ra.Pert = (const cx<R>*)p->Lam + (size_t)q.f0 * stride; ra.Lam = (cx<R>*)p->Lam + (size_t)q.f0 * stride; ra.stride_f = stride;
        ra.rx_lin = p->rx_lin; ra.mask = p->mask; ra.drec = (cx<R>*)p->drec + (size_t)q.f0 * nt * p->nm; ra.jv2 = jv2;
        ra.nt = nt; ra.nm = p->nm;
        {
            ProfScope ps(p, PC_RECEIVER, q.st);
            gn_receiver_kernel<R><<<dim3(nt, q.nf), 256, 0, q.st>>>(ra);
        }
        UST_LAUNCH_CHECK();
        UST_CUDA(cudaMemsetAsync((cx<R>*)p->Lam + (size_t)q.f0 * stride, 0, stride * q.nf * sizeof(cx<R>), q.st));
        {
            ProfScope ps(p, PC_RECEIVER, q.st);
            gn_scatter_kernel<R><<<dim3(nt, q.nf), 256, 0, q.st>>>(ra);
        }
        UST_LAUNCH_CHECK();
    }
    UST_TRY(sweeps_groups<R>(p, gs, (cx<R>*)p->Lam, stride, nt, 1));
    for (const Group& q : gs)
        for (int f = q.f0; f < q.f0 + q.nf; ++f) UST_TRY(ring_fix<R>(p, f, (cx<R>*)p->Lam + (size_t)f * stride, nt, 1, false, q.st));
    UST_TRY(join_groups(p, gs));
    GradArgs<R> ga;
    ga.U = (const cx<R>*)p->U; ga.Lam = (const cx<R>*)p->Lam; ga.stride_f = stride; ga.src_est = (const cx<R>*)p->src_est;
    ga.freqs = p->d_freqs; ga.slow = (const R*)p->slow_in; ga.grad = (R*)p->hv_out; ga.N = g.N; ga.nt = nt; ga.nfreq = nfreq;
    ga.kappa = nullptr; ga.grad_kappa = nullptr;
    const int blocks = (int)std::min<long long>((g.N + 7) / 8, (long long)p->num_sms * 8);
    {
        ProfScope ps(p, PC_GRADIENT, st);
        gradient_kernel<R, false><<<blocks, 256, 0, st>>>(ga);
    }
    UST_LAUNCH_CHECK();
    return 0;
}

template <typename F>
static int run_graphed(ust_plan* p, long long key, cudaStream_t user, F enqueue) {
    if (!p->use_graphs || p->prof) return enqueue(user);
    cudaStream_t gs = p->own_stream;
    auto it = p->graphs.find(key);
    if (it == p->graphs.end()) {
        const long long before = ust::g_launches;
        UST_CUDA(cudaStreamBeginCapture(gs, cudaStreamCaptureModeThreadLocal));
        int rc = enqueue(gs);
        cudaGraph_t graph = nullptr;
        cudaError_t e = cudaStreamEndCapture(gs, &graph);
        if (rc || e != cudaSuccess || !graph) {
            if (graph) cudaGraphDestroy(graph);
            if (!rc) set_error(std::string("CUDA graph capture failed: ") + cudaGetErrorString(e));
            cudaGetLastError();
            return 1;
        }
        ust_plan::GraphEntry ge;
        ge.launches = ust::g_launches - before;
        ust::g_launches = before;
        e = cudaGraphInstantiate(&ge.exec, graph, 0);
        cudaGraphDestroy(graph);
        if (e != cudaSuccess) { set_error(std::string("cudaGraphInstantiate failed: ") + cudaGetErrorString(e)); return 1; }
        it = p->graphs.emplace(key, ge).first;
    }
    UST_CUDA(cudaEventRecord(p->ev_in, user));
    UST_CUDA(cudaStreamWaitEvent(gs, p->ev_in, 0));
    UST_CUDA(cudaGraphLaunch(it->second.exec, gs));
    UST_CUDA(cudaEventRecord(p->ev_out, gs));
    UST_CUDA(cudaStreamWaitEvent(user, p->ev_out, 0));
    ust::g_launches += it->second.launches;
    return 0;
}

template <typename R>
static int fwi_impl(ust_plan* p, const void* slow, const void* rec, int nfreq, const double* freqs, const double* bde,
                    double* loss_dev, void* grad_dev, cudaStream_t st, const void* kappa = nullptr, void* grad_kappa_dev = nullptr) {
    const Geom& g = p->g;
    const bool lossy = kappa != nullptr;
    if (!p->acq_set) { set_error("ust_fwi_loss_grad: ust_plan_set_acquisition has not been called"); return 1; }
    if (!p->U) { set_error("ust_fwi_loss_grad: plan was created with fwi_buffers=0"); return 1; }
    if (p->nt > p->d.max_nrhs) { set_error("ust_fwi_loss_grad: nt exceeds plan max_nrhs"); return 1; }
    UST_TRY(upload_params(p, nfreq, freqs, bde, st));
    if (slow != p->slow_in) UST_CUDA(cudaMemcpyAsync(p->slow_in, slow, g.N * sizeof(R), cudaMemcpyDeviceToDevice, st));
    if (rec != p->rec_in) UST_CUDA(cudaMemcpyAsync(p->rec_in, rec, (size_t)nfreq * p->nt * p->nelem * sizeof(cx<R>), cudaMemcpyDeviceToDevice, st));
    if (lossy) UST_CUDA(cudaMemcpyAsync(p->kappa_in, kappa, g.N * sizeof(R), cudaMemcpyDeviceToDevice, st));
    const bool has_bde = bde != nullptr;
    const long long key = 1000LL * nfreq + (lossy ? 700 : 0) + (has_bde ? 1 : 0);
    p->gn_ok = false;
    UST_TRY(run_graphed(p, key, st, [&](cudaStream_t s_) { return fwi_enqueue<R>(p, nfreq, has_bde, s_, lossy); }));
    p->nfreq_cur = nfreq;
    p->factored = true;
    UST_CUDA(cudaMemcpyAsync(loss_dev, p->d_scal, sizeof(double), cudaMemcpyDeviceToDevice, st));
    UST_CUDA(cudaMemcpyAsync(grad_dev, p->grad_out, g.N * sizeof(R), cudaMemcpyDeviceToDevice, st));
    if (lossy) UST_CUDA(cudaMemcpyAsync(grad_kappa_dev, p->grad_kappa_out, g.N * sizeof(R), cudaMemcpyDeviceToDevice, st));
    p->fwi_done = true;
    p->lossy = lossy;
    p->gn_ok = !lossy;
    if (p->trace) return dump_update_trace(p, st);
    return 0;
}

template <typename R>
static int linesearch_impl(ust_plan* p, const void* sd, double* out2, cudaStream_t st) {
    const Geom& g = p->g;
    if (!p->factored || !p->fwi_done) { set_error("ust_ncg_linesearch: call ust_fwi_loss_grad first"); return 1; }
    if (p->lossy) {
        set_error("ust_ncg_linesearch: the plan holds a lossy model (ust_factor_lossy / ust_fwi_loss_grad_lossy) and the line search "
                  "assumes a real slowness; call ust_fwi_loss_grad first");
        return 1;
    }
    UST_CUDA(cudaMemcpyAsync(p->sd_in, sd, g.N * sizeof(R), cudaMemcpyDeviceToDevice, st));
    const long long key = 1000LL * p->nfreq_cur + 500;
    UST_TRY(run_graphed(p, key, st, [&](cudaStream_t s_) { return linesearch_enqueue<R>(p, s_); }));
    UST_CUDA(cudaMemcpyAsync(out2, p->d_scal + 2, 2 * sizeof(double), cudaMemcpyDeviceToDevice, st));
    return 0;
}

template <typename R>
static int gn_hvp_impl(ust_plan* p, const void* v, void* hv, double* jv2, void* jv, cudaStream_t st) {
    const Geom& g = p->g;
    if (!p->v_in) { set_error("ust_fwi_gn_hvp: plan was created with fwi_buffers=0"); return 1; }
    if (!p->factored || !p->fwi_done) { set_error("ust_fwi_gn_hvp: call ust_fwi_loss_grad first"); return 1; }
    if (p->lossy) {
        set_error("ust_fwi_gn_hvp: the plan holds a lossy model (ust_factor_lossy / ust_fwi_loss_grad_lossy) and the product "
                  "assumes a real slowness; call ust_fwi_loss_grad first");
        return 1;
    }
    if (!p->gn_ok) {
        set_error("ust_fwi_gn_hvp: the factors were replaced (ust_factor / ust_solve_helmholtz_host) after the last ust_fwi_loss_grad; "
                  "call ust_fwi_loss_grad again");
        return 1;
    }
    UST_CUDA(cudaMemcpyAsync(p->v_in, v, g.N * sizeof(R), cudaMemcpyDeviceToDevice, st));
    const long long key = 1000LL * p->nfreq_cur + 600;
    UST_TRY(run_graphed(p, key, st, [&](cudaStream_t s_) { return gn_hvp_enqueue<R>(p, s_); }));
    UST_CUDA(cudaMemcpyAsync(hv, p->hv_out, g.N * sizeof(R), cudaMemcpyDeviceToDevice, st));
    UST_CUDA(cudaMemcpyAsync(jv2, p->d_scal + 6, sizeof(double), cudaMemcpyDeviceToDevice, st));
    if (jv) UST_CUDA(cudaMemcpyAsync(jv, p->drec, (size_t)p->nfreq_cur * p->nt * p->nm * sizeof(cx<R>), cudaMemcpyDeviceToDevice, st));
    return 0;
}

template <typename R>
static int set_kernel_attrs() {
    UST_CUDA(cudaFuncSetAttribute(gj_pivot_kernel<R>, cudaFuncAttributeMaxDynamicSharedMemorySize,
                                  (int)std::max(gj_pivot_smem<R>(), sizeof(R) == 4 ? gj_pivot2_smem_bytes : gj_pivot_f64_smem_bytes)));
    if (sizeof(R) == 4) UST_CUDA(cudaFuncSetAttribute(gj_k0_kernel, cudaFuncAttributeMaxDynamicSharedMemorySize, (int)gj_pivot2_smem_bytes));
    if (sizeof(R) == 4) UST_CUDA(cudaFuncSetAttribute(schur_kernel<float>, cudaFuncAttributeMaxDynamicSharedMemorySize, (int)gj_pivot2_scratch_bytes));

    UST_CUDA(cudaFuncSetAttribute(gj_rowpanel_kernel<R>, cudaFuncAttributeMaxDynamicSharedMemorySize, (int)gj_rowpanel_smem<R>()));
    if (sizeof(R) == 4) {
        UST_CUDA(cudaFuncSetAttribute(tc2_sweep_gemm_kernel<true>, cudaFuncAttributeMaxDynamicSharedMemorySize, tc2::SMEM_BYTES));
        UST_CUDA(cudaFuncSetAttribute(tc2_sweep_gemm_kernel<false>, cudaFuncAttributeMaxDynamicSharedMemorySize, tc2::SMEM_BYTES));
        UST_CUDA(cudaFuncSetAttribute(tc2_gj_update_kernel, cudaFuncAttributeMaxDynamicSharedMemorySize, tc2::SMEM_BYTES_H));
        UST_CUDA(cudaFuncSetAttribute(tc2_gj_rowpanel_kernel, cudaFuncAttributeMaxDynamicSharedMemorySize, tc2::SMEM_BYTES_H));
        UST_CUDA(cudaFuncSetAttribute(tc2_gj_pivot_deep_kernel, cudaFuncAttributeMaxDynamicSharedMemorySize, tc2::SMEM_BYTES_H));
        UST_CUDA(cudaFuncSetAttribute(tc2_gj2_rowpanel_kernel, cudaFuncAttributeMaxDynamicSharedMemorySize, tc2::SMEM_BYTES_H));
        UST_CUDA(cudaFuncSetAttribute(tc2_gj2_update_kernel, cudaFuncAttributeMaxDynamicSharedMemorySize, tc2::SMEM_BYTES_H));
        UST_CUDA(cudaFuncSetAttribute(gj2_k0_kernel, cudaFuncAttributeMaxDynamicSharedMemorySize, (int)gj_pivot2_smem_bytes));
        UST_CUDA(cudaFuncSetAttribute(tc2h_test_gemm_kernel, cudaFuncAttributeMaxDynamicSharedMemorySize, tc2::SMEM_BYTES_H));
        UST_CUDA(cudaFuncSetAttribute(tc2_test_gemm_kernel<true>, cudaFuncAttributeMaxDynamicSharedMemorySize, tc2::SMEM_BYTES));
        UST_CUDA(cudaFuncSetAttribute(tc2_test_gemm_kernel<false>, cudaFuncAttributeMaxDynamicSharedMemorySize, tc2::SMEM_BYTES));
    }
    return 0;
}

#define DISPATCH(p, fn, ...) ((p)->d.dtype == UST_C64 ? fn<float>(__VA_ARGS__) : fn<double>(__VA_ARGS__))

struct IdtftCache { void* buf = nullptr; size_t cap = 0; cudaEvent_t ev = nullptr; bool used = false; };

template <typename R>
static int idtft_impl(const void* U, int nf, long long npix, const double* freqs, const double* resp, double df, const double* time, int nt,
                      void* out, cudaStream_t st) {
    const double PI = 3.14159265358979323846;
    std::vector<cx<R>> w((size_t)nt * nf);
    for (int t = 0; t < nt; ++t)
        for (int k = 0; k < nf; ++k) {
            const double ph = 2.0 * PI * freqs[k] * time[t], a = df * (resp ? resp[k] : 1.0);
            w[(size_t)t * nf + k] = cx<R>((R)(a * cos(ph)), (R)(a * sin(ph)));
        }
    int dev = 0;
    UST_CUDA(cudaGetDevice(&dev));
    static std::mutex mu;
    static std::map<int, IdtftCache> caches;
    std::lock_guard<std::mutex> lock(mu);
    IdtftCache& c = caches[dev];
    const size_t need = w.size() * sizeof(cx<R>);
    if (!c.ev) UST_CUDA(cudaEventCreateWithFlags(&c.ev, cudaEventDisableTiming));
    if (need > c.cap) {
        if (c.buf) { UST_CUDA(cudaEventSynchronize(c.ev)); cudaFree(c.buf); c.buf = nullptr; c.cap = 0; }
        UST_CUDA(cudaMalloc(&c.buf, need));
        c.cap = need;
    } else if (c.used) {
        UST_CUDA(cudaStreamWaitEvent(st, c.ev, 0));
    }
    cx<R>* wd = (cx<R>*)c.buf;
    UST_CUDA(cudaMemcpyAsync(wd, w.data(), need, cudaMemcpyHostToDevice, st));
    const size_t smem = (size_t)IDTFT_TT * nf * sizeof(cx<R>);
    if (smem > 48 * 1024) UST_CUDA(cudaFuncSetAttribute(idtft_kernel<R>, cudaFuncAttributeMaxDynamicSharedMemorySize, (int)smem));
    idtft_kernel<R><<<dim3((unsigned)((npix + 255) / 256), (unsigned)cdiv_i(nt, IDTFT_TT)), 256, smem, st>>>((const cx<R>*)U, wd, (cx<R>*)out, npix, nf, nt);
    UST_LAUNCH_CHECK();
    UST_CUDA(cudaEventRecord(c.ev, st));
    c.used = true;
    return 0;
}

extern "C" {

const char* ust_last_error(void) { return g_err.c_str(); }
const char* ust_version(void) { return "ustfwi 0.1 (sm_100a)"; }
int ust_idtft(int dtype, const void* U_dev, int nf, long long npix, const double* freqs, const double* resp, double df,
              const double* time, int nt, void* out_dev, void* stream) {
    if (!U_dev || !out_dev || !freqs || !time) { set_error("ust_idtft: null argument"); return 1; }
    if (nf < 1 || nt < 1 || npix < 1) { set_error("ust_idtft: empty problem"); return 1; }
    if ((size_t)IDTFT_TT * nf * (dtype == UST_C64 ? 8 : 16) > 200 * 1024) { set_error("ust_idtft: too many frequencies for one pass (split the stack)"); return 1; }
    if (dtype == UST_C64) return idtft_impl<float>(U_dev, nf, npix, freqs, resp, df, time, nt, out_dev, (cudaStream_t)stream);
    if (dtype == UST_C128) return idtft_impl<double>(U_dev, nf, npix, freqs, resp, df, time, nt, out_dev, (cudaStream_t)stream);
    set_error("ust_idtft: unknown dtype");
    return 1;
}

int ust_pack_f64_as_f32x2(const double* in_dev, float* out_dev, int n, void* stream) {
    if (!in_dev || !out_dev || n < 1) { set_error("ust_pack_f64_as_f32x2: bad arguments"); return 1; }
    pack_f32x2_kernel<<<cdiv_i(n, 128), 128, 0, (cudaStream_t)stream>>>(in_dev, out_dev, n);
    UST_LAUNCH_CHECK();
    return 0;
}

long long ust_launch_count(void) { return g_launches; }
void ust_launch_count_reset(void) { g_launches = 0; }

int ust_plan_create(const ust_plan_desc* d, ust_plan** out) {
    if (!d || !out) { set_error("ust_plan_create: null argument"); return 1; }
    if (d->nx < 5 || d->ny < 5) { set_error("ust_plan_create: grid must be at least 5x5"); return 1; }
    if (d->dtype != UST_C64 && d->dtype != UST_C128) { set_error("ust_plan_create: bad dtype"); return 1; }
    if (d->max_freq < 1 || d->max_nrhs < 1) { set_error("ust_plan_create: max_freq and max_nrhs must be >= 1"); return 1; }
    if (d->engine != UST_ENGINE_AUTO && d->engine != UST_ENGINE_SIMT && d->engine != UST_ENGINE_TC2) { set_error("ust_plan_create: unknown engine (AUTO, SIMT or TC2; the first tcgen05 engine, value 2, was removed)"); return 1; }
    if (d->engine == UST_ENGINE_TC2 && d->dtype != UST_C64) { set_error("ust_plan_create: the tensor-core engine is complex64 only (no FP64 tcgen05 kind)"); return 1; }
    int ndev = 0;
    UST_CUDA(cudaGetDeviceCount(&ndev));
    if (d->device < 0 || d->device >= ndev) { set_error("ust_plan_create: no such CUDA device"); return 1; }
    UST_CUDA(cudaSetDevice(d->device));
    ust_plan* p = new ust_plan();
    p->d = *d;
    Geom& g = p->g;
    g.Nx = d->nx; g.Ny = d->ny; g.nI = d->nx - 2; g.M = d->ny - 2;
    g.nP = ((g.nI + GJ_NB - 1) / GJ_NB) * GJ_NB;
    const bool want_tc2 = d->dtype == UST_C64 && (d->engine == UST_ENGINE_TC2 || d->engine == UST_ENGINE_AUTO);
    p->gj2 = false;
    if (const char* e = getenv("UST_GJ2")) p->gj2 = want_tc2 && atoi(e) != 0;
    if (const char* e = getenv("UST_NO_LOOKAHEAD")) { if (atoi(e) != 0) p->gj2 = false; }
    if (p->gj2) g.nP = ((g.nI + GJ_KB - 1) / GJ_KB) * GJ_KB;
    p->deep = false;
    if (const char* e = getenv("UST_DEEP")) p->deep = want_tc2 && !p->gj2 && atoi(e) != 0;
    p->fuse = false;
    if (const char* e = getenv("UST_FUSE_RP")) p->fuse = want_tc2 && !p->gj2 && atoi(e) != 0;
    if (const char* e = getenv("UST_NO_LOOKAHEAD")) { if (atoi(e) != 0) p->deep = false; }
    g.mid = g.M / 2;
    g.N = (long long)d->nx * d->ny;
    p->use_tc2 = d->dtype == UST_C64 && (d->engine == UST_ENGINE_TC2 || d->engine == UST_ENGINE_AUTO);
    if (const char* e = getenv("UST_TC2_BIAS_FIX")) p->bias_fix = (float)atof(e);
    if (const char* e = getenv("UST_TC2_GJ_DRAIN")) p->gj_drain = atoi(e);
    if (const char* e = getenv("UST_TC2_SWEEP_DRAIN")) p->sweep_drain = atoi(e);
    if (const char* e = getenv("UST_TC2_PREFETCH")) p->prefetch_cin = atoi(e);
    if (const char* e = getenv("UST_GROUPS")) p->ngroups = std::max(1, std::min(atoi(e), (int)ust_plan::MAX_GROUPS));
    p->t_ring = p->use_tc2;
    p->rsz = d->dtype == UST_C64 ? 4 : 8;
    p->csz = 2 * p->rsz;
    cudaDeviceProp prop;
    if (cudaGetDeviceProperties(&prop, d->device) == cudaSuccess) p->num_sms = prop.multiProcessorCount;
    const size_t bs = (size_t)g.nP * g.nP * p->csz;
    int rc = 0;
    rc |= dev_alloc(p, &p->exn, g.Nx * p->csz);
    rc |= dev_alloc(p, &p->rexh, g.Nx * p->csz);
    rc |= dev_alloc(p, &p->eyn, g.Ny * p->csz);
    rc |= dev_alloc(p, &p->reyh, g.Ny * p->csz);
    rc |= dev_alloc(p, (void**)&p->d_vminmax, 2 * sizeof(double));
    rc |= dev_alloc(p, (void**)&p->d_freqs, d->max_freq * sizeof(double));
    rc |= dev_alloc(p, (void**)&p->d_bde, 3 * d->max_freq * sizeof(double));
    rc |= dev_alloc(p, (void**)&p->d_scal, 8 * sizeof(double));
    rc |= dev_alloc(p, (void**)&p->d_status, sizeof(int));
    rc |= dev_alloc(p, (void**)&p->d_invv2, g.N * sizeof(double));
    rc |= dev_alloc(p, (void**)&p->d_sig2, 2 * g.N * sizeof(double));
    rc |= dev_alloc(p, &p->planes, (size_t)d->max_freq * 9 * g.N * p->csz);
    rc |= dev_alloc(p, &p->T, (size_t)d->max_freq * (p->t_ring ? 4 : g.M) * bs);
    if (!(d->dtype == UST_C64 && (d->engine == UST_ENGINE_TC2 || d->engine == UST_ENGINE_AUTO))) rc |= dev_alloc(p, &p->scratch, (size_t)2 * d->max_freq * bs);
    rc |= dev_alloc(p, &p->pbuf, (size_t)2 * d->max_freq * GJ_NB * GJ_NB * p->csz);
    rc |= dev_alloc(p, &p->W, (size_t)2 * d->max_freq * g.nP * d->max_nrhs * p->csz);
    rc |= dev_alloc(p, &p->vel, g.N * p->rsz);
    if (!rc && p->use_tc2) {
        p->kpad = ((g.nI + tc2::KC - 1) / tc2::KC) * tc2::KC;
        p->wp_stride = tc2::bplanes_elems(p->kpad, d->max_nrhs);
        const size_t tp_bytes = (size_t)d->max_freq * g.M * tc2::NPL_A * g.nP * g.nP * sizeof(uint16_t);
        const size_t wp_bytes = (size_t)2 * d->max_freq * p->wp_stride * sizeof(uint16_t);
        rc |= dev_alloc(p, (void**)&p->Tp, tp_bytes);
        rc |= dev_alloc(p, (void**)&p->Wp, wp_bytes);
        if (!rc && cudaMemset(p->Wp, 0, wp_bytes) != cudaSuccess) rc = 1;
        if (!rc) rc = tc2::make_aplane_maps(p->Tp, g.nP, (long long)d->max_freq * g.M, p->amaps);
        p->rp_stride = tc2::bplanes_elems(GJ_NB, g.nP);
        p->rp2_stride = tc2::bplanes_elems(GJ_KB, g.nP);
        const size_t nbmax = (size_t)2 * d->max_freq;
        const int cpw = p->gj2 ? GJ_KB : GJ_NB;
        rc |= dev_alloc(p, (void**)&p->Rp, (p->gj2 ? 1 : 2) * nbmax * (p->gj2 ? p->rp2_stride : p->rp_stride) * sizeof(uint16_t));
        rc |= dev_alloc(p, (void**)&p->gj_flags, 2 * GJ_MAXBLK * nbmax * sizeof(int));
        if (!rc && cudaMemset(p->gj_flags, 0, 2 * GJ_MAXBLK * nbmax * sizeof(int)) != cudaSuccess) rc = 1;
        rc |= dev_alloc(p, (void**)&p->Xp, 2 * nbmax * p->rp_stride * sizeof(uint16_t));
        rc |= dev_alloc(p, (void**)&p->Cp, 2 * nbmax * tc2::NPL_A * g.nP * cpw * sizeof(uint16_t));
        rc |= dev_alloc(p, (void**)&p->Pp, 2 * nbmax * tc2::NPL_A * GJ_NB * GJ_NB * sizeof(uint16_t));
        rc |= dev_alloc(p, &p->snap, 2 * nbmax * GJ_NB * GJ_NB * p->csz);
        if (p->deep) rc |= dev_alloc(p, (void**)&p->Rs, nbmax * p->rp_stride * sizeof(uint16_t));
        if (!rc && !p->gj2) rc = tc2::make_aplane_maps(p->Cp, g.nP, GJ_NB, (long long)(2 * nbmax), p->cmaps);
        if (!rc && p->gj2) rc = tc2::make_aplane_maps(p->Cp, g.nP, GJ_KB, (long long)(2 * nbmax), p->cmaps2);
        if (!rc) rc = tc2::make_aplane_maps(p->Pp, GJ_NB, GJ_NB, (long long)(2 * nbmax), p->pmaps);
    }
    if (d->fwi_buffers) {
        rc |= dev_alloc(p, &p->U, (size_t)d->max_freq * g.N * d->max_nrhs * p->csz);
        rc |= dev_alloc(p, &p->Lam, (size_t)d->max_freq * g.N * d->max_nrhs * p->csz);
        rc |= dev_alloc(p, &p->src_est, (size_t)d->max_freq * d->max_nrhs * p->csz);
        rc |= dev_alloc(p, &p->slow_in, g.N * p->rsz);
        rc |= dev_alloc(p, &p->grad_out, g.N * p->rsz);
        rc |= dev_alloc(p, &p->sd_in, g.N * p->rsz);
        rc |= dev_alloc(p, &p->v_in, g.N * p->rsz);
        rc |= dev_alloc(p, &p->hv_out, g.N * p->rsz);
        rc |= dev_alloc(p, &p->kappa_in, g.N * p->rsz);
        rc |= dev_alloc(p, &p->grad_kappa_out, g.N * p->rsz);
    }
    if (const char* e = getenv("UST_NO_GRAPHS")) p->use_graphs = atoi(e) == 0;
    if (const char* e = getenv("UST_NO_PDL")) ust::g_use_pdl = atoi(e) == 0;
    if (!rc && (cudaEventCreateWithFlags(&p->ev_in, cudaEventDisableTiming) != cudaSuccess ||
                cudaEventCreateWithFlags(&p->ev_out, cudaEventDisableTiming) != cudaSuccess)) {
        set_error("ust_plan_create: event creation failed");
        rc = 1;
    }
    if (!rc && cudaMallocHost((void**)&p->h_stage, 4 * d->max_freq * sizeof(double)) != cudaSuccess) {
        set_error("ust_plan_create: cudaMallocHost failed");
        rc = 1;
    }
    if (!rc && cudaStreamCreateWithFlags(&p->own_stream, cudaStreamNonBlocking) != cudaSuccess) {
        set_error("ust_plan_create: cudaStreamCreate failed");
        rc = 1;
    }
    if (!rc && cudaEventCreateWithFlags(&p->ev_fork, cudaEventDisableTiming) != cudaSuccess) rc = 1;
    for (int i = 1; i < ust_plan::MAX_GROUPS && !rc; ++i)
        if (cudaStreamCreateWithFlags(&p->side[i], cudaStreamNonBlocking) != cudaSuccess ||
            cudaEventCreateWithFlags(&p->ev_join[i], cudaEventDisableTiming) != cudaSuccess) {
            set_error("ust_plan_create: group stream / event creation failed");
            rc = 1;
        }
    if (!rc && (p->deep || d->dtype == UST_C128)) {
        int lo = 0, hi = 0;
        cudaDeviceGetStreamPriorityRange(&lo, &hi);
        for (int i = 0; i < ust_plan::MAX_GROUPS && !rc; ++i)
            if (cudaStreamCreateWithPriority(&p->pivst[i], cudaStreamNonBlocking, hi) != cudaSuccess ||
                cudaEventCreateWithFlags(&p->ev_upd[i], cudaEventDisableTiming) != cudaSuccess ||
                cudaEventCreateWithFlags(&p->ev_piv[i][0], cudaEventDisableTiming) != cudaSuccess ||
                cudaEventCreateWithFlags(&p->ev_piv[i][1], cudaEventDisableTiming) != cudaSuccess) {
                set_error("ust_plan_create: pivot stream / event creation failed");
                rc = 1;
            }
    }
    if (const char* e = getenv("UST_NO_LOOKAHEAD")) p->lookahead = atoi(e) == 0;
    if (const char* e = getenv("UST_NO_SCHUR_PIVOT")) p->schur_pivot0 = atoi(e) == 0;
    if (const char* e = getenv("UST_EXP")) p->exp = atoi(e);
    if (const char* e = getenv("UST_PDL_MIN_BATCH")) p->pdl_min_batch = atoi(e);
    if (const char* e = getenv("UST_KSPLIT")) p->ksplit_ok = atoi(e);
    if (const char* e = getenv("UST_TC2_TRACE_UPDATE")) {
        if (sscanf(e, "%d,%d", &p->trace_step, &p->trace_k) == 2 && cudaMalloc((void**)&p->trace, 19 * 1024 * sizeof(unsigned long long)) == cudaSuccess)
            cudaMemset(p->trace, 0, 19 * 1024 * sizeof(unsigned long long));
    }
    if (!rc) rc = (d->dtype == UST_C64) ? set_kernel_attrs<float>() : set_kernel_attrs<double>();
    if (!rc && cudaMemset(p->d_status, 0, sizeof(int)) != cudaSuccess) rc = 1;
    if (rc) {
        std::string keep = g_err;
        ust_plan_destroy(p);
        set_error(keep.empty() ? "ust_plan_create: allocation failed" : keep);
        return 1;
    }
    *out = p;
    return 0;
}

int ust_plan_destroy(ust_plan* p) {
    if (!p) return 0;
    cudaSetDevice(p->d.device);
    cudaDeviceSynchronize();
    void* ptrs[] = {p->exn, p->rexh, p->eyn, p->reyh, p->d_vminmax, p->d_freqs, p->d_bde, p->d_scal, p->d_status, p->d_invv2, p->d_sig2, p->planes,
                    p->T, p->scratch, p->W, p->pbuf, p->Tp, p->Wp, p->Rp, p->Cp, p->Xp, p->Pp, p->Rs, p->gj_flags, p->snap, p->vel, p->U, p->Lam, p->src_est, p->Xh, p->src_lin, p->rx_lin, p->mask,
                    p->slow_h2d, p->rec_h2d, p->grad_d2h, p->kappa_h2d, p->grad_kappa_d2h};
    for (void* q : ptrs)
        if (q) cudaFree(q);
    drop_graphs(p);
    for (void* q : {p->slow_in, p->rec_in, p->grad_out, p->sd_in, p->v_in, p->hv_out, p->drec, p->kappa_in, p->grad_kappa_out})
        if (q) cudaFree(q);
    if (p->ev_in) cudaEventDestroy(p->ev_in);
    if (p->ev_out) cudaEventDestroy(p->ev_out);
    if (p->h_stage) cudaFreeHost(p->h_stage);
    if (p->own_stream) cudaStreamDestroy(p->own_stream);
    if (p->ev_fork) cudaEventDestroy(p->ev_fork);
    for (int i = 0; i < ust_plan::MAX_GROUPS; ++i) {
        if (p->side[i]) cudaStreamDestroy(p->side[i]);
        if (p->ev_join[i]) cudaEventDestroy(p->ev_join[i]);
        if (p->pivst[i]) cudaStreamDestroy(p->pivst[i]);
        if (p->ev_upd[i]) cudaEventDestroy(p->ev_upd[i]);
        for (int j = 0; j < 2; ++j)
            if (p->ev_piv[i][j]) cudaEventDestroy(p->ev_piv[i][j]);
    }

    for (cudaEvent_t e : p->ev) cudaEventDestroy(e);
    delete p;
    return 0;
}

size_t ust_plan_device_bytes(const ust_plan* p) { return p ? p->bytes : 0; }

int ust_plan_set_groups(ust_plan* p, int ngroups) {
    UST_TRY(check_plan(p));
    if (ngroups < 1 || ngroups > ust_plan::MAX_GROUPS) { set_error("ust_plan_set_groups: 1 <= ngroups <= 8"); return 1; }
    if (ngroups == p->ngroups) return 0;
    UST_CUDA(cudaSetDevice(p->d.device));
    UST_CUDA(cudaDeviceSynchronize());
    drop_graphs(p);
    p->ngroups = ngroups;
    return 0;
}

int ust_plan_set_grid(ust_plan* p, const double* x, const double* y, double a0, double L) {
    UST_TRY(check_plan(p));
    if (!x || !y || !(L > 0)) { set_error("ust_plan_set_grid: bad arguments"); return 1; }
    UST_CUDA(cudaSetDevice(p->d.device));
    UST_CUDA(cudaDeviceSynchronize());
    drop_graphs(p);
    return p->d.dtype == UST_C64 ? set_grid_impl<float>(p, x, y, a0, L) : set_grid_impl<double>(p, x, y, a0, L);
}

int ust_plan_set_acquisition(ust_plan* p, int nt, const int32_t* src_lin, int nelem, const int32_t* rx_lin, int nm,
                             const int32_t* mask) {
    UST_TRY(check_plan(p));
    if (nt < 1 || nelem < 1 || nm < 1 || !src_lin || !rx_lin || !mask) { set_error("ust_plan_set_acquisition: bad arguments"); return 1; }
    const Geom& g = p->g;
    auto interior = [&](int lin) {
        int y = lin / g.Nx, x = lin % g.Nx;
        return lin >= 0 && lin < g.N && x > 0 && y > 0 && x < g.Nx - 1 && y < g.Ny - 1;
    };
    for (int i = 0; i < nt; ++i)
        if (!interior(src_lin[i])) { set_error("ust_plan_set_acquisition: a source lies on or outside the Dirichlet ring"); return 1; }
    for (int i = 0; i < nelem; ++i)
        if (!interior(rx_lin[i])) { set_error("ust_plan_set_acquisition: a receiver lies on or outside the Dirichlet ring"); return 1; }
    for (long long i = 0; i < (long long)nt * nm; ++i)
        if (mask[i] < 0 || mask[i] >= nelem) { set_error("ust_plan_set_acquisition: mask index out of range"); return 1; }
    UST_CUDA(cudaSetDevice(p->d.device));
    UST_CUDA(cudaDeviceSynchronize());
    drop_graphs(p);
    p->fwi_done = false;
    p->gn_ok = false;
    for (int** q : {&p->src_lin, &p->rx_lin, &p->mask})
        if (*q) { cudaFree(*q); *q = nullptr; }
    if (p->rec_in) { cudaFree(p->rec_in); p->rec_in = nullptr; }
    if (p->rec_h2d) { cudaFree(p->rec_h2d); p->rec_h2d = nullptr; }
    if (p->drec) { cudaFree(p->drec); p->drec = nullptr; }
    if (p->d.fwi_buffers) UST_CUDA(cudaMalloc(&p->rec_in, (size_t)p->d.max_freq * nt * nelem * p->csz));
    if (p->d.fwi_buffers) UST_CUDA(cudaMalloc(&p->drec, (size_t)p->d.max_freq * nt * nm * p->csz));
    UST_CUDA(cudaMalloc((void**)&p->src_lin, nt * sizeof(int)));
    UST_CUDA(cudaMalloc((void**)&p->rx_lin, nelem * sizeof(int)));
    UST_CUDA(cudaMalloc((void**)&p->mask, (size_t)nt * nm * sizeof(int)));
    UST_CUDA(cudaMemcpy(p->src_lin, src_lin, nt * sizeof(int), cudaMemcpyHostToDevice));
    UST_CUDA(cudaMemcpy(p->rx_lin, rx_lin, nelem * sizeof(int), cudaMemcpyHostToDevice));
    UST_CUDA(cudaMemcpy(p->mask, mask, (size_t)nt * nm * sizeof(int), cudaMemcpyHostToDevice));
    p->nt = nt; p->nelem = nelem; p->nm = nm; p->acq_set = true;
    p->onehot_ok = cdiv_i(nt, 128) <= 8;
    for (int i = 0; i < 8; ++i) { p->first_row[i] = 32767; p->last_row[i] = -1; }
    if (p->onehot_ok)
        for (int i = 0; i < nt; ++i) {
            const short r = (short)(src_lin[i] / g.Nx - 1);
            short& lo = p->first_row[i / 128]; short& hi = p->last_row[i / 128];
            lo = std::min(lo, r); hi = std::max(hi, r);
        }
    return 0;
}

int ust_factor(ust_plan* p, const void* vel_dev, int nfreq, const double* freqs, const double* bde, void* stream) {
    UST_TRY(check_plan(p));
    if (!vel_dev || !freqs) { set_error("ust_factor: null argument"); return 1; }
    UST_CUDA(cudaSetDevice(p->d.device));
    const int rc = DISPATCH(p, factor_impl, p, vel_dev, nfreq, freqs, bde, (cudaStream_t)stream);
    if (!rc && p->trace) return dump_update_trace(p, (cudaStream_t)stream);
    return rc;
}

int ust_factor_lossy(ust_plan* p, const void* vel_dev, const void* kappa_dev, int nfreq, const double* freqs, const double* bde, void* stream) {
    UST_TRY(check_plan(p));
    if (!vel_dev || !kappa_dev || !freqs) { set_error("ust_factor_lossy: null argument (kappa_dev is required)"); return 1; }
    UST_CUDA(cudaSetDevice(p->d.device));
    return DISPATCH(p, factor_impl, p, vel_dev, nfreq, freqs, bde, (cudaStream_t)stream, kappa_dev);
}

int ust_solve(ust_plan* p, int ifreq, void* X, int nrhs, int adjoint, void* stream) {
    UST_TRY(check_plan(p));
    if (!X) { set_error("ust_solve: null argument"); return 1; }
    UST_CUDA(cudaSetDevice(p->d.device));
    return DISPATCH(p, solve_impl, p, ifreq, X, nrhs, adjoint, (cudaStream_t)stream);
}

int ust_solve_helmholtz_host(ust_plan* p, const void* vel_host, const void* src_host, void* out_host, int nrhs, double f,
                             const double* bde, int adjoint, int refactor) {
    UST_TRY(check_plan(p));
    if (!src_host || !out_host) { set_error("ust_solve_helmholtz_host: null argument"); return 1; }
    if (nrhs < 1 || nrhs > p->d.max_nrhs) { set_error("ust_solve_helmholtz_host: nrhs exceeds plan max_nrhs"); return 1; }
    UST_CUDA(cudaSetDevice(p->d.device));
    const Geom& g = p->g;
    cudaStream_t st = p->own_stream;
    if (!p->Xh) UST_TRY(dev_alloc(p, &p->Xh, (size_t)g.N * p->d.max_nrhs * p->csz));
    if (refactor || !p->factored) {
        if (!vel_host) { set_error("ust_solve_helmholtz_host: vel required to factorise"); return 1; }
        UST_CUDA(cudaMemcpyAsync(p->vel, vel_host, g.N * p->rsz, cudaMemcpyHostToDevice, st));
        UST_TRY(DISPATCH(p, factor_impl, p, p->vel, 1, &f, bde, st));
    }
    const size_t bytes = (size_t)g.N * nrhs * p->csz;
    UST_CUDA(cudaMemcpyAsync(p->Xh, src_host, bytes, cudaMemcpyHostToDevice, st));
    UST_TRY(DISPATCH(p, solve_impl, p, 0, p->Xh, nrhs, adjoint, st));
    UST_CUDA(cudaMemcpyAsync(out_host, p->Xh, bytes, cudaMemcpyDeviceToHost, st));
    int status = 0;
    UST_CUDA(cudaMemcpyAsync(&status, p->d_status, sizeof(int), cudaMemcpyDeviceToHost, st));
    UST_CUDA(cudaStreamSynchronize(st));
    if (status) { set_error("ust_solve_helmholtz_host: a block inversion met a zero / non-finite pivot (singular operator)"); return 2; }
    return 0;
}

int ust_fwi_loss_grad(ust_plan* p, const void* slow, const void* rec, int nfreq, const double* freqs, const double* bde,
                      double* loss_dev, void* grad_dev, void* stream) {
    UST_TRY(check_plan(p));
    if (!slow || !rec || !freqs || !loss_dev || !grad_dev) { set_error("ust_fwi_loss_grad: null argument"); return 1; }
    UST_CUDA(cudaSetDevice(p->d.device));
    return DISPATCH(p, fwi_impl, p, slow, rec, nfreq, freqs, bde, loss_dev, grad_dev, (cudaStream_t)stream);
}

static int fwi_host(ust_plan* p, const char* name, const void* slow_host, const void* kappa_host, const void* rec_host, int nfreq,
                    const double* freqs, const double* bde, double* loss_host, void* grad_host, void* grad_kappa_host) {
    if (!p->acq_set) { set_error(std::string(name) + ": ust_plan_set_acquisition has not been called"); return 1; }
    UST_CUDA(cudaSetDevice(p->d.device));
    const Geom& g = p->g;
    cudaStream_t st = p->own_stream;
    if (nfreq < 1 || nfreq > p->d.max_freq) { set_error(std::string(name) + ": nfreq out of range"); return 1; }
    const size_t rec_bytes = (size_t)p->d.max_freq * p->nt * p->nelem * p->csz;
    if (!p->slow_h2d) UST_TRY(dev_alloc(p, &p->slow_h2d, g.N * p->rsz));
    if (!p->grad_d2h) UST_TRY(dev_alloc(p, &p->grad_d2h, g.N * p->rsz));
    if (!p->rec_h2d) UST_CUDA(cudaMalloc(&p->rec_h2d, rec_bytes));
    if (kappa_host && !p->kappa_h2d) UST_TRY(dev_alloc(p, &p->kappa_h2d, g.N * p->rsz));
    if (kappa_host && !p->grad_kappa_d2h) UST_TRY(dev_alloc(p, &p->grad_kappa_d2h, g.N * p->rsz));
    UST_CUDA(cudaMemcpyAsync(p->slow_h2d, slow_host, g.N * p->rsz, cudaMemcpyHostToDevice, st));
    UST_CUDA(cudaMemcpyAsync(p->rec_h2d, rec_host, (size_t)nfreq * p->nt * p->nelem * p->csz, cudaMemcpyHostToDevice, st));
    if (kappa_host) UST_CUDA(cudaMemcpyAsync(p->kappa_h2d, kappa_host, g.N * p->rsz, cudaMemcpyHostToDevice, st));
    UST_TRY(DISPATCH(p, fwi_impl, p, p->slow_h2d, p->rec_h2d, nfreq, freqs, bde, p->d_scal, p->grad_d2h, st,
                     kappa_host ? p->kappa_h2d : nullptr, p->grad_kappa_d2h));
    UST_CUDA(cudaMemcpyAsync(loss_host, p->d_scal, sizeof(double), cudaMemcpyDeviceToHost, st));
    UST_CUDA(cudaMemcpyAsync(grad_host, p->grad_d2h, g.N * p->rsz, cudaMemcpyDeviceToHost, st));
    if (kappa_host) UST_CUDA(cudaMemcpyAsync(grad_kappa_host, p->grad_kappa_d2h, g.N * p->rsz, cudaMemcpyDeviceToHost, st));
    int status = 0;
    UST_CUDA(cudaMemcpyAsync(&status, p->d_status, sizeof(int), cudaMemcpyDeviceToHost, st));
    UST_CUDA(cudaStreamSynchronize(st));
    if (status) {
// ... 215 lines not shown
```

Before: 28840.

## Add persistent Gauss-Jordan update kernel overlapping next tile loads with epilogue

Adds a persistent tensor-core update kernel in which each CTA loops over many GEMM tiles, possibly with two thread groups per CTA. While the current tile's epilogue stages and stores, the next tile's operand load is issued. It becomes the default path when there is no ping-pong snapshot and no fused row-panel work. The aim is to remove per-tile launch and prologue cost and to hide epilogue latency, at the price of more shared memory per CTA and new mbarrier phase logic that could hurt occupancy or correctness.

After: 27140 (median of 6 runs). 0.941x the previous value.

```diff
diff --git a/waveforminversionust_b200/csrc/factor.cuh b/waveforminversionust_b200/csrc/factor.cuh
--- a/waveforminversionust_b200/csrc/factor.cuh
+++ b/waveforminversionust_b200/csrc/factor.cuh
@@ -954,6 +954,78 @@
     gj_rowpanel_tile(a, k, z, row, freq, blockIdx.x, bias_fix, &pmap, tc2_smem);
 }
 
+__device__ __forceinline__ void gj_lookahead_pivot(const FactorArgs<float>& a, int k, int z, float bias_fix, int rp_next, const CUtensorMap* cmap,
+                                                   unsigned char* tc2_smem) {
+    static_assert(tc2::CH_LD == GJ_NB + 1, "pivot body reads the staged tile with row stride GJ_NB + 1");
+    const int kb = k + 1, nP = a.g.nP;
+    const int row = chain_row(a.g, a.phase, z, a.step);
+    if (row < 0 || (a.exp & 2)) {
+        if (row >= 0 && rp_next && threadIdx.x == 0) atomicExch(gj_flag(a, 0, kb, z), 1);
+        pdl_wait();
+        return;
+    }
+    tc2::Tc2Tile t;
+    tc2::tile_no_emit(t);
+    t.bplanes = gj_rp(a, k, z);
+    t.amat = (k & 1) * a.nbmax + a.zb0 + z;
+    const cx<float>* S1 = a.snap + ((size_t)(a.pp ? (kb & 1) * a.nbmax : 0) + a.zb0 + z) * GJ_NB * GJ_NB;
+    t.Cin = S1 - (size_t)(kb * GJ_NB) * GJ_NB - kb * GJ_NB; t.ldcin = GJ_NB;
+    t.Cout = nullptr; t.ldc = nP; t.keep = 1;
+    t.M = nP; t.N = nP; t.K = GJ_NB; t.Mstore = nP;
+    t.m0 = (kb >> 1) * tc2::TM; t.n0 = kb * GJ_NB;
+    t.mask_lo = 0; t.mask_hi = 0;
+    t.skip_lo = (kb ^ 1) * GJ_NB; t.skip_hi = t.skip_lo + GJ_NB;
+    t.sgn = -1.f; t.bias_fix = bias_fix; t.drain_every = a.gj_drain;
+    const bool traced = a.trace && a.step == a.trace_step && k == a.trace_k && z < 24;
+    if (traced) {
+        t.trace = a.trace + 16 * (1000 + z);
+        if (threadIdx.x == 0) { unsigned smid; asm volatile("mov.u32 %0, %%smid;" : "=r"(smid)); a.trace[16 * 1024 + 1000 + z] = smid; }
+    }
+    tc2::cgemm_tile_h(t, cmap, tc2_smem);
+    __syncthreads();
+    if (a.exp & 1) {
+        if (rp_next && threadIdx.x == 0) atomicExch(gj_flag(a, 0, kb, z), 1);
+        return;
+    }
+    unsigned char* smem_al = tc2_smem + ((128u - (tc::smem_u32(tc2_smem) & 127u)) & 127u);
+    cx<float>* blk = reinterpret_cast<cx<float>*>(smem_al) + (size_t)(kb & 1) * GJ_NB * tc2::CH_LD;
+    cx<float>* scr = reinterpret_cast<cx<float>*>(smem_al) + (size_t)tc2::TM * tc2::CH_LD;
+    static_assert((size_t)tc2::TM * tc2::CH_LD * sizeof(cx<float>) + gj_pivot2_scratch_bytes <= (size_t)tc2::STAGES_H * tc2::STAGE_H,
+                  "pivot scratch must fit behind the staging tile inside the operand ring");
+    FactorArgs<float> a2 = a;
+    if (a.pp) a2.Pp = a.Pp + (size_t)(kb & 1) * a.nbmax * tc2::NPL_A * GJ_NB * GJ_NB;
+    gj_pivot_blocked(a2, z, blk, scr, threadIdx.x, traced ? a.trace + 18 * 1024 + 16 * z : nullptr);
+    if (traced && threadIdx.x == 0) a.trace[17 * 1024 + 1000 + z] = tc2::gtime();
+    if (rp_next) {
+        __threadfence();
+        __syncthreads();
+        if (threadIdx.x == 0) atomicExch(gj_flag(a, 0, kb, z), 1);
+    }
+}
+
+__device__ __forceinline__ void gj_update_tile(const FactorArgs<float>& a, int k, int z, int row, int mt, int nt, float bias_fix, tc2::Tc2Tile& t) {
+    const int nP = a.g.nP, nblk = nP / GJ_NB;
+    const int freq = a.f0 + chain_freq(a.phase, z);
+    tc2::tile_no_emit(t);
+    t.bplanes = gj_rp(a, k, z);
+    t.amat = (k & 1) * a.nbmax + a.zb0 + z;
+    t.Cin = gj_buffer(a, z, freq, row, k); t.ldcin = nP;
+    t.Cout = gj_buffer(a, z, freq, row, k + 1); t.ldc = nP;
+    t.M = nP; t.N = nP; t.K = GJ_NB; t.Mstore = nP;
+    t.m0 = mt * tc2::TM; t.n0 = nt * tc2::TNH;
+    t.mask_lo = k * GJ_NB; t.mask_hi = (k + 1) * GJ_NB;
+    t.skip_lo = k * GJ_NB; t.skip_hi = (k + 1) * GJ_NB;
+    t.sgn = -1.f;
+    t.bias_fix = bias_fix;
+    t.drain_every = a.gj_drain;
+    gj_emit_a(a, t, z, freq, row, k, 0);
+    if (k + 1 < nblk) {
+        t.eb_planes = a.Xp + ((size_t)((k + 1) & 1) * a.nbmax + a.zb0 + z) * a.rp_stride;
+        t.eb_m_lo = (k + 1) * GJ_NB; t.eb_id_lo = (k + 1) * GJ_NB; t.eb_id_hi = (k + 2) * GJ_NB;
+    }
+    t.prefetch_cin = a.prefetch_cin;
+}
+
 __global__ void __launch_bounds__(tc2::NUM_THREADS_H, 2)
 tc2_gj_update_kernel(FactorArgs<float> a, int k, float bias_fix, int pivot_next, int rp_next, const __grid_constant__ CUtensorMap cmap,
                      const __grid_constant__ CUtensorMap pmap) {
@@ -963,53 +1035,7 @@
     int bid = blockIdx.x;
     if (pivot_next) {
         if (bid < a.nbatch) {
-            {
-                static_assert(tc2::CH_LD == GJ_NB + 1, "pivot body reads the staged tile with row stride GJ_NB + 1");
-                const int z = bid, kb = k + 1, nP = a.g.nP;
-                const int row = chain_row(a.g, a.phase, z, a.step);
-                if (row < 0 || (a.exp & 2)) {
-                    if (row >= 0 && rp_next && threadIdx.x == 0) atomicExch(gj_flag(a, 0, kb, z), 1);
-                    pdl_wait();
-                    return;
-                }
-                tc2::Tc2Tile t;
-                tc2::tile_no_emit(t);
-                t.bplanes = gj_rp(a, k, z);
-                t.amat = (k & 1) * a.nbmax + a.zb0 + z;
-                const cx<float>* S1 = a.snap + ((size_t)(a.pp ? (kb & 1) * a.nbmax : 0) + a.zb0 + z) * GJ_NB * GJ_NB;
-                t.Cin = S1 - (size_t)(kb * GJ_NB) * GJ_NB - kb * GJ_NB; t.ldcin = GJ_NB;
-                t.Cout = nullptr; t.ldc = nP; t.keep = 1;
-                t.M = nP; t.N = nP; t.K = GJ_NB; t.Mstore = nP;
-                t.m0 = (kb >> 1) * tc2::TM; t.n0 = kb * GJ_NB;
-                t.mask_lo = 0; t.mask_hi = 0;
-                t.skip_lo = (kb ^ 1) * GJ_NB; t.skip_hi = t.skip_lo + GJ_NB;
-                t.sgn = -1.f; t.bias_fix = bias_fix; t.drain_every = a.gj_drain;
-                const bool traced = a.trace && a.step == a.trace_step && k == a.trace_k && z < 24;
-                if (traced) {
-                    t.trace = a.trace + 16 * (1000 + z);
-                    if (threadIdx.x == 0) { unsigned smid; asm volatile("mov.u32 %0, %%smid;" : "=r"(smid)); a.trace[16 * 1024 + 1000 + z] = smid; }
-                }
-                tc2::cgemm_tile_h(t, &cmap, tc2_smem);
-                __syncthreads();
-                if (a.exp & 1) {
-                    if (rp_next && threadIdx.x == 0) atomicExch(gj_flag(a, 0, kb, z), 1);
-                    return;
-                }
-                unsigned char* smem_al = tc2_smem + ((128u - (tc::smem_u32(tc2_smem) & 127u)) & 127u);
-                cx<float>* blk = reinterpret_cast<cx<float>*>(smem_al) + (size_t)(kb & 1) * GJ_NB * tc2::CH_LD;
-                cx<float>* scr = reinterpret_cast<cx<float>*>(smem_al) + (size_t)tc2::TM * tc2::CH_LD;
-                static_assert((size_t)tc2::TM * tc2::CH_LD * sizeof(cx<float>) + gj_pivot2_scratch_bytes <= (size_t)tc2::STAGES_H * tc2::STAGE_H,
-                              "pivot scratch must fit behind the staging tile inside the operand ring");
-                FactorArgs<float> a2 = a;
-                if (a.pp) a2.Pp = a.Pp + (size_t)(kb & 1) * a.nbmax * tc2::NPL_A * GJ_NB * GJ_NB;
-                gj_pivot_blocked(a2, z, blk, scr, threadIdx.x, traced ? a.trace + 18 * 1024 + 16 * z : nullptr);
-                if (traced && threadIdx.x == 0) a.trace[17 * 1024 + 1000 + z] = tc2::gtime();
-                if (rp_next) {
-                    __threadfence();
-                    __syncthreads();
-                    if (threadIdx.x == 0) atomicExch(gj_flag(a, 0, kb, z), 1);
-                }
-            }
+            gj_lookahead_pivot(a, k, bid, bias_fix, rp_next, &cmap, tc2_smem);
             return;
         }
         bid -= a.nbatch;
@@ -1055,30 +1081,12 @@
     }
     const int row = chain_row(a.g, a.phase, z, a.step);
     if (row < 0) { pdl_wait(); return; }
-    const int freq = (a.f0 + chain_freq(a.phase, z));
     tc2::Tc2Tile t;
-    tc2::tile_no_emit(t);
-    t.bplanes = gj_rp(a, k, z);
-    t.amat = (k & 1) * a.nbmax + a.zb0 + z;
-    t.Cin = gj_buffer(a, z, freq, row, k); t.ldcin = nP;
-    t.Cout = gj_buffer(a, z, freq, row, k + 1); t.ldc = nP;
-    t.M = nP; t.N = nP; t.K = GJ_NB; t.Mstore = nP;
-    t.m0 = mt * tc2::TM; t.n0 = nt * TW;
-    t.mask_lo = k * GJ_NB; t.mask_hi = (k + 1) * GJ_NB;
-    t.skip_lo = k * GJ_NB; t.skip_hi = (k + 1) * GJ_NB;
-    t.sgn = -1.f;
-    t.bias_fix = bias_fix;
-    t.drain_every = a.gj_drain;
-    gj_emit_a(a, t, z, freq, row, k, 0);
-    if (k + 1 < nblk) {
-        t.eb_planes = a.Xp + ((size_t)((k + 1) & 1) * a.nbmax + a.zb0 + z) * a.rp_stride;
-        t.eb_m_lo = (k + 1) * GJ_NB; t.eb_id_lo = (k + 1) * GJ_NB; t.eb_id_hi = (k + 2) * GJ_NB;
-    }
+    gj_update_tile(a, k, z, row, mt, nt, bias_fix, t);
     if (a.trace && a.step == a.trace_step && k == a.trace_k && bid < 900) {
         t.trace = a.trace + 16 * bid;
         if (threadIdx.x == 0) { unsigned smid; asm volatile("mov.u32 %0, %%smid;" : "=r"(smid)); a.trace[16 * 1024 + bid] = smid; }
     }
-    t.prefetch_cin = a.prefetch_cin;
     const int kk = k + 2;
     const bool snap_next = a.pp && kk < nblk && t.m0 == (kk >> 1) * tc2::TM && t.n0 == kk * GJ_NB;
     if (snap_next) t.keep = 1;
@@ -1099,6 +1107,36 @@
         __syncthreads();
         if (threadIdx.x == 0) atomicAdd(gj_flag(a, 1, k + 1, z), 1);
     }
+}
+
+__global__ void __launch_bounds__(tc2::NUM_THREADS_P, 1)
+tc2_gj_update_persistent_kernel(FactorArgs<float> a, int k, float bias_fix, int pivot_next, const __grid_constant__ CUtensorMap cmap) {
+    extern __shared__ __align__(1024) unsigned char tc2_smem[];
+    pdl_trigger();
+    int bid = blockIdx.x, nctas = gridDim.x;
+    if (pivot_next) {
+        if (bid < a.nbatch) {
+            if (threadIdx.x >= tc2::NUM_THREADS_H) return;
+            gj_lookahead_pivot(a, k, bid, bias_fix, 0, &cmap, tc2_smem);
+            return;
+        }
+        bid -= a.nbatch;
+        nctas -= a.nbatch;
+    }
+    const int nP = a.g.nP;
+    const int tiles_m = (nP + tc2::TM - 1) / tc2::TM, tiles = (nP + tc2::TNH - 1) / tc2::TNH;
+    const int per_row = a.nbatch * tiles, total = per_row * tiles_m;
+    const int first = ((k + 1) >> 1) < tiles_m ? (k + 1) >> 1 : 0;
+    const int ntiles = bid < total ? (total - bid + nctas - 1) / nctas : 0;
+    auto chain_of = [&](int j) { return ((bid + j * nctas) % per_row) / tiles; };
+    auto live = [&](int j) { return chain_row(a.g, a.phase, chain_of(j), a.step) >= 0; };
+    auto make = [&](int j, tc2::Tc2Tile& t) {
+        const int idx = bid + j * nctas, mt_local = idx / per_row, rem = idx % per_row;
+        const int z = rem / tiles, nt = rem % tiles;
+        const int mt = mt_local == 0 ? first : (mt_local <= first ? mt_local - 1 : mt_local);
+        gj_update_tile(a, k, z, chain_row(a.g, a.phase, z, a.step), mt, nt, bias_fix, t);
+    };
+    tc2::cgemm_tiles_h_persistent(ntiles, live, make, &cmap, tc2_smem);
 }
 
 __global__ void __launch_bounds__(tc2::NUM_THREADS_H, 2)
diff --git a/waveforminversionust_b200/csrc/gemm_tc2h.cuh b/waveforminversionust_b200/csrc/gemm_tc2h.cuh
--- a/waveforminversionust_b200/csrc/gemm_tc2h.cuh
+++ b/waveforminversionust_b200/csrc/gemm_tc2h.cuh
@@ -26,6 +26,131 @@
         for (int i = 0; i < 2 * STAGES_H + 3; ++i) asm volatile("mbarrier.inval.shared::cta.b64 [%0];" ::"r"(bar_base + 8u * i) : "memory");
     }
     __syncthreads();
+}
+
+__device__ __forceinline__ void tile_h_stage(uint32_t tmem_d2, int r, int cg, float bias, const float (&acc_re)[32], const float (&acc_im)[32],
+                                             cx<float>* stage) {
+    typedef cx<float> C;
+#pragma unroll
+    for (int h = 0; h < 4; ++h) {
+        uint32_t vr[8], vi[8];
+        tmem_ld8(tmem_d2 + (uint32_t)(32 * cg + 8 * h), vr);
+        tmem_ld8(tmem_d2 + (uint32_t)(TNH + 32 * cg + 8 * h), vi);
+        asm volatile("tcgen05.wait::ld.sync.aligned;" ::: "memory");
+#pragma unroll
+        for (int j = 0; j < 8; ++j) {
+            const float ar = acc_re[8 * h + j], ai = acc_im[8 * h + j];
+            const float cr = fmaf(ar, bias, __uint_as_float(vr[j]));
+            const float ci = fmaf(ai, bias, __uint_as_float(vi[j]));
+            stage[(size_t)r * CH_LD + 32 * cg + 8 * h + j] = C(ar + cr, ai + ci);
+        }
+    }
+}
+
+template <class Sync>
+__device__ __forceinline__ void tile_h_store(const Tc2Tile& tl, cx<float>* stage, int tid, Sync sync, unsigned long long* trace) {
+    typedef cx<float> C;
+    const int warp = tid >> 5, lane = tid & 31;
+    const bool emit = tl.ea_planes != nullptr || tl.eb_planes != nullptr || tl.keep;
+    const bool vec_ok = ((tl.ldc & 1) == 0) && ((((uintptr_t)tl.Cout) & 15) == 0) && (tl.n0 % 2 == 0) &&
+                        (!tl.Cin || (((tl.ldcin & 1) == 0) && ((((uintptr_t)tl.Cin) & 15) == 0)));
+    if (vec_ok && tl.n0 + TNH <= tl.N) {
+        constexpr int RPW = TM / NUM_WARPS_H;
+        float4 cin[RPW];
+        unsigned live = 0;
+        const int nloc = lane * 2, n = tl.n0 + nloc;
+#pragma unroll
+        for (int j = 0; j < RPW; ++j) {
+            const int m = tl.m0 + warp + NUM_WARPS_H * j;
+            const bool lv = m < tl.Mstore && !(m >= tl.skip_lo && m < tl.skip_hi);
+            live |= (lv ? 1u : 0u) << j;
+            cin[j] = make_float4(0.f, 0.f, 0.f, 0.f);
+            if (lv && tl.Cin) cin[j] = *reinterpret_cast<const float4*>(tl.Cin + (size_t)m * tl.ldcin + n);
+        }
+        const bool z0 = n >= tl.mask_lo && n < tl.mask_hi, z1 = n + 1 >= tl.mask_lo && n + 1 < tl.mask_hi;
+#pragma unroll
+        for (int j = 0; j < RPW; ++j) {
+            const int rr = warp + NUM_WARPS_H * j;
+            const int m = tl.m0 + rr;
+            if (!((live >> j) & 1u)) continue;
+            const C a0 = stage[(size_t)rr * CH_LD + nloc], a1 = stage[(size_t)rr * CH_LD + nloc + 1];
+            float4 c = cin[j];
+            if (z0) { c.x = 0.f; c.y = 0.f; }
+            if (z1) { c.z = 0.f; c.w = 0.f; }
+            c.x += tl.sgn * a0.re; c.y += tl.sgn * a0.im; c.z += tl.sgn * a1.re; c.w += tl.sgn * a1.im;
+            if (tl.Cout) *reinterpret_cast<float4*>(tl.Cout + (size_t)m * tl.ldc + n) = c;
+            if (emit) { stage[(size_t)rr * CH_LD + nloc] = C(c.x, c.y); stage[(size_t)rr * CH_LD + nloc + 1] = C(c.z, c.w); }
+        }
+    } else {
+        for (int rr = warp; rr < TM; rr += NUM_WARPS_H) {
+            const int m = tl.m0 + rr;
+            if (m >= tl.Mstore || (m >= tl.skip_lo && m < tl.skip_hi)) continue;
+            const int nloc = lane * 2, n = tl.n0 + nloc;
+            if (n >= tl.N) continue;
+            const C a0 = stage[(size_t)rr * CH_LD + nloc], a1 = stage[(size_t)rr * CH_LD + nloc + 1];
+            C c0 = cxzero<float>(), c1 = cxzero<float>();
+            if (tl.Cin) {
+                const C* ci = tl.Cin + (size_t)m * tl.ldcin + n;
+                c0 = ci[0];
+                if (n + 1 < tl.N) c1 = ci[1];
+                if (n >= tl.mask_lo && n < tl.mask_hi) c0 = cxzero<float>();
+                if (n + 1 >= tl.mask_lo && n + 1 < tl.mask_hi) c1 = cxzero<float>();
+            }
+            c0.re += tl.sgn * a0.re; c0.im += tl.sgn * a0.im;
+            c1.re += tl.sgn * a1.re; c1.im += tl.sgn * a1.im;
+            if (tl.Cout) {
+                C* co = tl.Cout + (size_t)m * tl.ldc + n;
+                co[0] = c0;
+                if (n + 1 < tl.N) co[1] = c1;
+            }
+            if (emit) { stage[(size_t)rr * CH_LD + nloc] = c0; stage[(size_t)rr * CH_LD + nloc + 1] = c1; }
+        }
+    }
+    if (trace && warp == 3 && lane == 0) trace[12] = gtime();
+    if (emit) {
+        sync();
+        if (tl.eb_planes && tl.eb_m_lo >= tl.m0 && tl.eb_m_lo < tl.m0 + TM) {
+            const int r0 = tl.eb_m_lo - tl.m0;
+#pragma unroll
+            for (int h = 0; h < 2; ++h) {
+                const int e = tid + NUM_THREADS_H * h;
+                const int nloc = e & (TNH - 1), kg = e >> 6;
+                const int n = tl.n0 + nloc;
+                float re[8], im[8];
+#pragma unroll
+                for (int c = 0; c < 8; ++c) {
+                    C v = stage[(size_t)(r0 + 8 * kg + c) * CH_LD + nloc];
+                    if (n >= tl.eb_id_lo && n < tl.eb_id_hi) v = C((n - tl.eb_id_lo == 8 * kg + c) ? 1.f : 0.f, 0.f);
+                    if (n >= tl.N) v = cxzero<float>();
+                    re[c] = v.re; im[c] = v.im;
+                }
+                const int ech = tl.eb_chunks > 0 ? tl.eb_chunks : 64 / KC;
+                uint16_t* chunk = tl.eb_planes + ((size_t)(n / TN) * ech + tl.eb_chunk0 + (kg >> 1)) * (B_STAGE / 2);
+                store_b8(chunk, n % TN, kg & 1, re, im);
+            }
+        }
+        if (tl.ea_planes) {
+            const int lo = tl.ea_n_lo > tl.n0 ? tl.ea_n_lo : tl.n0;
+            const int hi = tl.ea_n_hi < tl.n0 + TNH ? tl.ea_n_hi : tl.n0 + TNH;
+            const int nJ = hi > lo ? (hi - lo) >> 3 : 0;
+            for (int e = tid; e < nJ * TM; e += NUM_THREADS_H) {
+                const int rr = e & (TM - 1), jj = e >> 7;
+                const int m = tl.m0 + rr;
+                if (m >= tl.Mstore || (m >= tl.skip_lo && m < tl.skip_hi)) continue;
+                const int n8 = lo + 8 * jj;
+                const int tr = m + tl.ea_row_off, tcol = n8 - tl.ea_col_off;
+                float re[8], im[8];
+#pragma unroll
+                for (int c = 0; c < 8; ++c) {
+                    C v = stage[(size_t)rr * CH_LD + (n8 - tl.n0) + c];
+                    if (tr >= tl.ea_zero_from || tcol + c >= tl.ea_zero_from || n8 + c >= tl.N) v = cxzero<float>();
+                    re[c] = v.re; im[c] = v.im;
+                }
+                uint16_t* dst = tl.ea_planes + ((size_t)(tr >> 3) * tl.ea_nbc + (tcol >> 3)) * 64 + (tr & 7) * 8;
+                store_a8(dst, tl.ea_plane_elems, re, im);
+            }
+        }
+    }
 }
 
 __device__ __forceinline__ void cgemm_tile_h(const Tc2Tile& t_in, const CUtensorMap* amap, unsigned char* smem_raw) {
@@ -179,24 +304,7 @@
     if (warp == 3) TC2_TRACE(10);
     asm volatile("tcgen05.fence::after_thread_sync;" ::: "memory");
     C* stage = reinterpret_cast<C*>(smem_al);
-    {
-        const int r = q * 32 + lane;
-        const float bias = t.bias_fix * (float)D;
-#pragma unroll
-        for (int h = 0; h < 4; ++h) {
-            uint32_t vr[8], vi[8];
-            tmem_ld8(D2 + lane_addr + (uint32_t)(32 * cg + 8 * h), vr);
-            tmem_ld8(D2 + lane_addr + (uint32_t)(TNH + 32 * cg + 8 * h), vi);
-            asm volatile("tcgen05.wait::ld.sync.aligned;" ::: "memory");
-#pragma unroll
-            for (int j = 0; j < 8; ++j) {
-                const float ar = acc_re[8 * h + j], ai = acc_im[8 * h + j];
-                const float cr = fmaf(ar, bias, __uint_as_float(vr[j]));
-                const float ci = fmaf(ai, bias, __uint_as_float(vi[j]));
-                stage[(size_t)r * CH_LD + 32 * cg + 8 * h + j] = C(ar + cr, ai + ci);
-            }
-        }
-    }
+    tile_h_stage(D2 + lane_addr, q * 32 + lane, cg, t.bias_fix * (float)D, acc_re, acc_im, stage);
     if (warp == 3) TC2_TRACE(11);
     asm volatile("tcgen05.fence::before_thread_sync;" ::: "memory");
     __syncthreads();
@@ -206,109 +314,192 @@
     }
     if (warp == 3) TC2_TRACE(15);
     const Tc2Tile tl = *t_sh;
-    const bool emit = tl.ea_planes != nullptr || tl.eb_planes != nullptr || tl.keep;
-    const bool vec_ok = ((tl.ldc & 1) == 0) && ((((uintptr_t)tl.Cout) & 15) == 0) && (tl.n0 % 2 == 0) &&
-                        (!tl.Cin || (((tl.ldcin & 1) == 0) && ((((uintptr_t)tl.Cin) & 15) == 0)));
-    if (vec_ok && tl.n0 + TNH <= tl.N) {
-        constexpr int RPW = TM / NUM_WARPS_H;
-        float4 cin[RPW];
-        unsigned live = 0;
-        const int nloc = lane * 2, n = tl.n0 + nloc;
-#pragma unroll
-        for (int j = 0; j < RPW; ++j) {
-            const int m = tl.m0 + warp + NUM_WARPS_H * j;
-            const bool lv = m < tl.Mstore && !(m >= tl.skip_lo && m < tl.skip_hi);
-            live |= (lv ? 1u : 0u) << j;
-            cin[j] = make_float4(0.f, 0.f, 0.f, 0.f);
-            if (lv && tl.Cin) cin[j] = *reinterpret_cast<const float4*>(tl.Cin + (size_t)m * tl.ldcin + n);
-        }
-        const bool z0 = n >= tl.mask_lo && n < tl.mask_hi, z1 = n + 1 >= tl.mask_lo && n + 1 < tl.mask_hi;
-#pragma unroll
-        for (int j = 0; j < RPW; ++j) {
-            const int rr = warp + NUM_WARPS_H * j;
-            const int m = tl.m0 + rr;
-            if (!((live >> j) & 1u)) continue;
-            const C a0 = stage[(size_t)rr * CH_LD + nloc], a1 = stage[(size_t)rr * CH_LD + nloc + 1];
-            float4 c = cin[j];
-            if (z0) { c.x = 0.f; c.y = 0.f; }
-            if (z1) { c.z = 0.f; c.w = 0.f; }
-            c.x += tl.sgn * a0.re; c.y += tl.sgn * a0.im; c.z += tl.sgn * a1.re; c.w += tl.sgn * a1.im;
-            if (tl.Cout) *reinterpret_cast<float4*>(tl.Cout + (size_t)m * tl.ldc + n) = c;
-            if (emit) { stage[(size_t)rr * CH_LD + nloc] = C(c.x, c.y); stage[(size_t)rr * CH_LD + nloc + 1] = C(c.z, c.w); }
-        }
-    } else {
-        for (int rr = warp; rr < TM; rr += NUM_WARPS_H) {
-            const int m = tl.m0 + rr;
-            if (m >= tl.Mstore || (m >= tl.skip_lo && m < tl.skip_hi)) continue;
-            const int nloc = lane * 2, n = tl.n0 + nloc;
-            if (n >= tl.N) continue;
-            const C a0 = stage[(size_t)rr * CH_LD + nloc], a1 = stage[(size_t)rr * CH_LD + nloc + 1];
-            C c0 = cxzero<float>(), c1 = cxzero<float>();
-            if (tl.Cin) {
-                const C* ci = tl.Cin + (size_t)m * tl.ldcin + n;
-                c0 = ci[0];
-                if (n + 1 < tl.N) c1 = ci[1];
-                if (n >= tl.mask_lo && n < tl.mask_hi) c0 = cxzero<float>();
-                if (n + 1 >= tl.mask_lo && n + 1 < tl.mask_hi) c1 = cxzero<float>();
-            }
-            c0.re += tl.sgn * a0.re; c0.im += tl.sgn * a0.im;
-            c1.re += tl.sgn * a1.re; c1.im += tl.sgn * a1.im;
-            if (tl.Cout) {
-                C* co = tl.Cout + (size_t)m * tl.ldc + n;
-                co[0] = c0;
-                if (n + 1 < tl.N) co[1] = c1;
-            }
-            if (emit) { stage[(size_t)rr * CH_LD + nloc] = c0; stage[(size_t)rr * CH_LD + nloc + 1] = c1; }
-        }
-    }
-    if (warp == 3) TC2_TRACE(12);
-    if (emit) {
-        __syncthreads();
-        if (tl.eb_planes && tl.eb_m_lo >= tl.m0 && tl.eb_m_lo < tl.m0 + TM) {
-            const int r0 = tl.eb_m_lo - tl.m0;
-#pragma unroll
-            for (int h = 0; h < 2; ++h) {
-                const int e = tid + NUM_THREADS_H * h;
-                const int nloc = e & (TNH - 1), kg = e >> 6;
-                const int n = tl.n0 + nloc;
-                float re[8], im[8];
-#pragma unroll
-                for (int c = 0; c < 8; ++c) {
-                    C v = stage[(size_t)(r0 + 8 * kg + c) * CH_LD + nloc];
-                    if (n >= tl.eb_id_lo && n < tl.eb_id_hi) v = C((n - tl.eb_id_lo == 8 * kg + c) ? 1.f : 0.f, 0.f);
-                    if (n >= tl.N) v = cxzero<float>();
-                    re[c] = v.re; im[c] = v.im;
-                }
-                const int ech = tl.eb_chunks > 0 ? tl.eb_chunks : 64 / KC;
-                uint16_t* chunk = tl.eb_planes + ((size_t)(n / TN) * ech + tl.eb_chunk0 + (kg >> 1)) * (B_STAGE / 2);
-                store_b8(chunk, n % TN, kg & 1, re, im);
-            }
-        }
-        if (tl.ea_planes) {
-            const int lo = tl.ea_n_lo > tl.n0 ? tl.ea_n_lo : tl.n0;
-            const int hi = tl.ea_n_hi < tl.n0 + TNH ? tl.ea_n_hi : tl.n0 + TNH;
-            const int nJ = hi > lo ? (hi - lo) >> 3 : 0;
-            for (int e = tid; e < nJ * TM; e += NUM_THREADS_H) {
-                const int rr = e & (TM - 1), jj = e >> 7;
-                const int m = tl.m0 + rr;
-                if (m >= tl.Mstore || (m >= tl.skip_lo && m < tl.skip_hi)) continue;
-                const int n8 = lo + 8 * jj;
-                const int tr = m + tl.ea_row_off, tcol = n8 - tl.ea_col_off;
-                float re[8], im[8];
-#pragma unroll
-                for (int c = 0; c < 8; ++c) {
-                    C v = stage[(size_t)rr * CH_LD + (n8 - tl.n0) + c];
-                    if (tr >= tl.ea_zero_from || tcol + c >= tl.ea_zero_from || n8 + c >= tl.N) v = cxzero<float>();
-                    re[c] = v.re; im[c] = v.im;
-                }
-                uint16_t* dst = tl.ea_planes + ((size_t)(tr >> 3) * tl.ea_nbc + (tcol >> 3)) * 64 + (tr & 7) * 8;
-                store_a8(dst, tl.ea_plane_elems, re, im);
-            }
-        }
-    }
+    tile_h_store(tl, stage, tid, [] { __syncthreads(); }, t_in.trace);
     if (warp == 3) TC2_TRACE(13);
     if (warp == 2) TC2_TRACE(14);
 }
 
-}
-}
+constexpr int NUM_THREADS_P = 2 * NUM_THREADS_H;
+constexpr int NK_P = 4;
+constexpr int RING_P = STAGES_H * STAGE_H;
+__host__ __device__ constexpr int smem_bytes_p(int ng) { return ng * RING_P + 128 + ng * (128 + 384); }
+static_assert(TM * CH_LD * 8 <= 2 * STAGE_H, "a group's staging tile must leave the third stage of its ring free");
+static_assert(smem_bytes_p(2) <= 227 * 1024, "one CTA of two groups per SM");
+static_assert(2 * (smem_bytes_p(1) + 1024) <= 228 * 1024, "two CTAs of one group per SM");
+static_assert(smem_bytes_p(1) >= SMEM_BYTES_H, "CTAs of the same launch may run cgemm_tile_h in this shared memory");
+
+template <class Live, class Make>
+__device__ __forceinline__ void cgemm_tiles_h_persistent(int ntiles, Live live, Make make, const CUtensorMap* amap, unsigned char* smem_raw) {
+    typedef cx<float> C;
+    const int tid = threadIdx.x, warp = tid >> 5, lane = tid & 31;
+    const int ng = blockDim.x / NUM_THREADS_H, g = warp >> 3, gw = warp & 7, gtid = tid & (NUM_THREADS_H - 1);
+    const uint32_t tmem_cols = (uint32_t)ng * TMEM_COLS_H;
+    if (tid == 0) asm volatile("prefetch.tensormap [%0];" ::"l"((uint64_t)amap) : "memory");
+    const uint32_t smem_base = (smem_u32(smem_raw) + 127u) & ~127u;
+    unsigned char* smem_al = smem_raw + (smem_base - smem_u32(smem_raw));
+    const uint32_t ring = smem_base + g * RING_P;
+    const int tail = ng * RING_P;
+    const uint32_t bar_base = smem_base + tail + 128u * g;
+    auto full_bar = [&](int s) { return bar_base + 8u * s; };
+    auto empty_bar = [&](int s) { return bar_base + 8u * (STAGES_H + s); };
+    const uint32_t d1_full = bar_base + 8u * (2 * STAGES_H);
+    const uint32_t d1_empty = d1_full + 8u;
+    const uint32_t d2_full = d1_full + 16u;
+    const uint32_t tmem_slot = smem_base + tail + 120u;
+    volatile uint32_t* tmem_slot_ptr = reinterpret_cast<volatile uint32_t*>(smem_al + tail + 120);
+    Tc2Tile* t_sh = reinterpret_cast<Tc2Tile*>(smem_al + tail + 128 * ng + 384 * g);
+    C* stage = reinterpret_cast<C*>(smem_al + g * RING_P);
+    auto gsync = [g] { asm volatile("bar.sync %0, %1;" ::"r"(1 + g), "r"(NUM_THREADS_H) : "memory"); };
+
+    if (gw == 2 && lane == 0) {
+        for (int s = 0; s < STAGES_H; ++s) { mbar_init(full_bar(s), 1); mbar_init(empty_bar(s), 2); }
+        mbar_init(d1_full, 1);
+        mbar_init(d1_empty, NUM_WARPS_H);
+        mbar_init(d2_full, 1);
+        asm volatile("fence.mbarrier_init.release.cluster;" ::: "memory");
+    }
+    if (warp == 2) {
+        __syncwarp();
+        asm volatile("tcgen05.alloc.cta_group::1.sync.aligned.shared::cta.b32 [%0], %1;" ::"r"(tmem_slot), "r"(tmem_cols) : "memory");
+        asm volatile("tcgen05.relinquish_alloc_permit.cta_group::1.sync.aligned;" ::: "memory");
+    }
+    asm volatile("tcgen05.fence::before_thread_sync;" ::: "memory");
+    __syncthreads();
+    asm volatile("tcgen05.fence::after_thread_sync;" ::: "memory");
+    const uint32_t tmem_acc = *tmem_slot_ptr;
+    pdl_wait();
+    const uint32_t D1 = tmem_acc + (uint32_t)(g * TMEM_COLS_H), D2 = D1 + 2 * TNH;
+
+    auto load_chunk = [&](const Tc2Tile& tt, int c) {
+        const int s = (c + 2) % STAGES_H;
+        const uint32_t sa = ring + s * STAGE_H, sb = sa + A_STAGE;
+        const unsigned char* bc = reinterpret_cast<const unsigned char*>(tt.bplanes) + ((size_t)(tt.n0 / TN) * NK_P + c) * B_STAGE + ((tt.n0 % TN) / TNH) * 2048;
+        mbar_expect_tx_e(full_bar(s), STAGE_H);
+        tma_load_5d_e(sa, amap, full_bar(s), 0, (c * KC) >> 3, tt.m0 >> 3, 0, tt.amat);
+#pragma unroll
+        for (int p = 0; p < NPL_B; ++p) {
+            bulk_load_e(sb + p * BH_PLANE, bc + p * B_PLANE, 2048, full_bar(s));
+            bulk_load_e(sb + p * BH_PLANE + 2048, bc + p * B_PLANE + 4096, 2048, full_bar(s));
+        }
+    };
+    const uint32_t id1 = IDESC_N128, id2 = IDESC_N64 | IDESC_ANEG, id3 = IDESC_N64;
+    uint64_t dAr[3], dAi[3], dB[3], dBi[3];
+#pragma unroll
+    for (int i = 0; i < 3; ++i) {
+        dAr[i] = make_desc(ring + i * A_PLANE, 128u, 256u);
+        dAi[i] = make_desc(ring + (3 + i) * A_PLANE, 128u, 256u);
+        dB[i] = make_desc(ring + A_STAGE + i * BH_PLANE, 128u, 256u);
+        dBi[i] = make_desc(ring + A_STAGE + i * BH_PLANE + (TNH / 8) * 256, 128u, 256u);
+    }
+    auto issue = [&](uint32_t d, uint64_t so, int i, int j, uint32_t acc_first) {
+        umma_e(d, dAr[i] + so, dB[j] + so, id1, acc_first);
+        umma_e(d, dAi[i] + so, dBi[j] + so, id2, 1u);
+        umma_e(d + TNH, dAi[i] + so, dB[j] + so, id3, 1u);
+    };
+    auto next_live = [&](int j) { while (j < ntiles && !live(j)) j += ng; return j; };
+
+    const int q = warp & 3, cg = gw >> 2;
+    const uint32_t lane_addr = ((uint32_t)(q * 32)) << 16;
+    uint32_t d1n = 0;
+    int j = next_live(g);
+    if (j < ntiles) {
+        if (gtid == 0) make(j, *t_sh);
+        gsync();
+        if (gw == 0) load_chunk(*t_sh, 0);
+    }
+    for (uint32_t it = 0; j < ntiles; ++it) {
+        const Tc2Tile& t = *t_sh;
+        if (gw == 2) { load_chunk(t, 1); load_chunk(t, 2); }
+        if (t.Cin && gtid >= 128 && t.prefetch_cin) {
+            const int rr = gtid - 128, m = t.m0 + rr;
+            const int ncols = t.N - t.n0 < TNH ? t.N - t.n0 : TNH;
+            if (m < t.Mstore && !(m >= t.skip_lo && m < t.skip_hi) && ncols > 0 && ((ncols * 8) & 15) == 0 && ((t.ldcin & 1) == 0) && ((t.n0 & 1) == 0))
+                asm volatile("cp.async.bulk.prefetch.L2.global [%0], %1;" ::"l"((uint64_t)(t.Cin + (size_t)m * t.ldcin + t.n0)), "r"((uint32_t)(ncols * 8)) : "memory");
+        }
+        const int D = t.drain_every < 1 ? 1 : (t.drain_every > NK_P ? NK_P : t.drain_every);
+        float acc_re[32], acc_im[32];
+#pragma unroll
+        for (int i = 0; i < 32; ++i) { acc_re[i] = 0.f; acc_im[i] = 0.f; }
+        for (int c = 0; c < NK_P; ++c) {
+            const int s = (c + 2) % STAGES_H;
+            if (gw < 2) {
+                const uint64_t so = (uint64_t)((uint32_t)(s * STAGE_H) >> 4);
+                mbar_wait(full_bar(s), s == 2 ? (c == 3 ? 1u : 0u) : (it & 1u));
+                if (gw == 0) {
+                    if (c > 0 && c % D == 0) mbar_wait(d1_empty, (d1n - 1u) & 1u);
+                    asm volatile("tcgen05.fence::after_thread_sync;" ::: "memory");
+                    issue(D1, so, 0, 0, c % D == 0 ? 0u : 1u);
+                    if ((c + 1) % D == 0 || c == NK_P - 1) umma_commit_e(d1_full);
+                    umma_commit_e(empty_bar(s));
+                } else {
+                    asm volatile("tcgen05.fence::after_thread_sync;" ::: "memory");
+                    issue(D2, so, 0, 1, c > 0 ? 1u : 0u);
+                    issue(D2, so, 1, 0, 1u);
+                    issue(D2, so, 0, 2, 1u);
+                    issue(D2, so, 2, 0, 1u);
+                    issue(D2, so, 1, 1, 1u);
+                    umma_commit_e(empty_bar(s));
+                    if (c == NK_P - 1) umma_commit_e(d2_full);
+                }
+                __syncwarp();
+            }
+            if ((c + 1) % D == 0 || c == NK_P - 1) {
+                mbar_wait(d1_full, d1n & 1u);
+                asm volatile("tcgen05.fence::after_thread_sync;" ::: "memory");
+#pragma unroll
+                for (int h = 0; h < 4; ++h) {
+                    uint32_t vr[8], vi[8];
+                    tmem_ld8(D1 + lane_addr + (uint32_t)(32 * cg + 8 * h), vr);
+                    tmem_ld8(D1 + lane_addr + (uint32_t)(TNH + 32 * cg + 8 * h), vi);
+                    asm volatile("tcgen05.wait::ld.sync.aligned;" ::: "memory");
+                    if (h == 3) {
+                        asm volatile("tcgen05.fence::before_thread_sync;" ::: "memory");
+                        __syncwarp();
+                        if (lane == 0) mbar_arrive(d1_empty);
+                    }
+#pragma unroll
+                    for (int i = 0; i < 8; ++i) {
+                        acc_re[8 * h + i] += __uint_as_float(vr[i]);
+                        acc_im[8 * h + i] += __uint_as_float(vi[i]);
+                    }
+                }
+                ++d1n;
+            }
+            if (gw == 0 && c == 0) {
+                mbar_wait(empty_bar(2), 0u);
+                load_chunk(t, 3);
+            }
+        }
+        mbar_wait(d2_full, it & 1u);
+        asm volatile("tcgen05.fence::after_thread_sync;" ::: "memory");
+        const int jn = next_live(j + ng);
+        if (gw == 0 && jn < ntiles) {
+            Tc2Tile tn;
+            make(jn, tn);
+            mbar_wait(empty_bar(2), 1u);
+            load_chunk(tn, 0);
+        }
+        tile_h_stage(D2 + lane_addr, q * 32 + lane, cg, t.bias_fix * (float)D, acc_re, acc_im, stage);
+        asm volatile("tcgen05.fence::before_thread_sync;" ::: "memory");
+        gsync();
+        const Tc2Tile tl = *t_sh;
+        tile_h_store(tl, stage, gtid, gsync, nullptr);
+        asm volatile("fence.proxy.async.shared::cta;" ::: "memory");
+        gsync();
+        j = jn;
+        if (j < ntiles) {
+            if (gtid == 0) make(j, *t_sh);
+            gsync();
+        }
+    }
+    asm volatile("tcgen05.fence::before_thread_sync;" ::: "memory");
+    __syncthreads();
+    if (warp == 2) {
+        asm volatile("tcgen05.fence::after_thread_sync;" ::: "memory");
+        asm volatile("tcgen05.dealloc.cta_group::1.sync.aligned.b32 %0, %1;" ::"r"(tmem_acc), "r"(tmem_cols) : "memory");
+    }
+}
+
+
+}
+}
diff --git a/waveforminversionust_b200/csrc/ustfwi.cu b/waveforminversionust_b200/csrc/ustfwi.cu
--- a/waveforminversionust_b200/csrc/ustfwi.cu
+++ b/waveforminversionust_b200/csrc/ustfwi.cu
@@ -43,6 +43,7 @@
     cudaEvent_t ev_upd[MAX_GROUPS] = {}, ev_piv[MAX_GROUPS][2] = {};
     uint16_t* Rs = nullptr;
     bool fuse = false;
+    bool persist = true;
     int* gj_flags = nullptr;
     uint16_t *Tp = nullptr, *Wp = nullptr;
     void* snap = nullptr;
@@ -179,6 +180,8 @@
     return 0;
 }
 
+static bool persist_split() { const char* e = getenv("UST_PERSIST_SPLIT"); return e && atoi(e) != 0; }
+static int persist_ng() { const char* e = getenv("UST_PERSIST_NG"); return e && atoi(e) == 1 ? 1 : 2; }
 template <typename R>
 static int gj_invert_batch(ust_plan* p, int phase, int step, int f0, int nf, cudaStream_t st, int gidx) {
     const Geom& g = p->g;
@@ -283,8 +286,18 @@
                     const int pivot_next = (la && k + 1 < nblk) ? 1 : 0;
                     const int rp_next = (a.fuse && k + 1 < nblk && !(p->exp & 4)) ? 1 : 0;
                     ProfScope ps(p, PC_GJ_UPDATE, st);
-                    UST_CUDA(launch_pdl(tc2_gj_update_kernel, dim3(nbatch * tiles * tiles_h + (pivot_next ? nbatch : 0) + (rp_next ? nbatch * tiles_h : 0)), dim3(tc2::NUM_THREADS_H),
-                                        tc2::SMEM_BYTES_H, st, a, k, p->bias_fix, pivot_next, rp_next, p->cmaps[0], p->pmaps[0]));
+                    if (p->persist && !a.pp && !rp_next) {
+                        const int ntiles = nbatch * tiles * tiles_h;
+                        const int G = persist_split() ? p->active_groups : 1;
+                        const int ng = persist_ng();
+                        const int slots = (3 - ng) * p->num_sms;
+                        const int P = std::max(1, std::min(ntiles, (slots - G * (pivot_next ? nbatch : 0)) / G));
+                        UST_CUDA(launch_pdl(tc2_gj_update_persistent_kernel, dim3(P + (pivot_next ? nbatch : 0)), dim3(ng * tc2::NUM_THREADS_H),
+                                            tc2::smem_bytes_p(ng), st, a, k, p->bias_fix, pivot_next, p->cmaps[0]));
+                    } else {
+                        UST_CUDA(launch_pdl(tc2_gj_update_kernel, dim3(nbatch * tiles * tiles_h + (pivot_next ? nbatch : 0) + (rp_next ? nbatch * tiles_h : 0)), dim3(tc2::NUM_THREADS_H),
+                                            tc2::SMEM_BYTES_H, st, a, k, p->bias_fix, pivot_next, rp_next, p->cmaps[0], p->pmaps[0]));
+                    }
                     UST_LAUNCH_CHECK();
                 }
                 if (deep && k + 2 < nblk) UST_TRY(pivot_deep(k + 2));
@@ -843,6 +856,7 @@
         UST_CUDA(cudaFuncSetAttribute(tc2_sweep_gemm_kernel<true>, cudaFuncAttributeMaxDynamicSharedMemorySize, tc2::SMEM_BYTES));
         UST_CUDA(cudaFuncSetAttribute(tc2_sweep_gemm_kernel<false>, cudaFuncAttributeMaxDynamicSharedMemorySize, tc2::SMEM_BYTES));
         UST_CUDA(cudaFuncSetAttribute(tc2_gj_update_kernel, cudaFuncAttributeMaxDynamicSharedMemorySize, tc2::SMEM_BYTES_H));
+        UST_CUDA(cudaFuncSetAttribute(tc2_gj_update_persistent_kernel, cudaFuncAttributeMaxDynamicSharedMemorySize, tc2::smem_bytes_p(2)));
         UST_CUDA(cudaFuncSetAttribute(tc2_gj_rowpanel_kernel, cudaFuncAttributeMaxDynamicSharedMemorySize, tc2::SMEM_BYTES_H));
         UST_CUDA(cudaFuncSetAttribute(tc2_gj_pivot_deep_kernel, cudaFuncAttributeMaxDynamicSharedMemorySize, tc2::SMEM_BYTES_H));
         UST_CUDA(cudaFuncSetAttribute(tc2_gj2_rowpanel_kernel, cudaFuncAttributeMaxDynamicSharedMemorySize, tc2::SMEM_BYTES_H));
@@ -946,6 +960,7 @@
     p->fuse = false;
     if (const char* e = getenv("UST_FUSE_RP")) p->fuse = want_tc2 && !p->gj2 && atoi(e) != 0;
     if (const char* e = getenv("UST_NO_LOOKAHEAD")) { if (atoi(e) != 0) p->deep = false; }
+    if (const char* e = getenv("UST_PERSIST")) p->persist = atoi(e) != 0;
     g.mid = g.M / 2;
     g.N = (long long)d->nx * d->ny;
     p->use_tc2 = d->dtype == UST_C64 && (d->engine == UST_ENGINE_TC2 || d->engine == UST_ENGINE_AUTO);
```
